# adamchang2000/DenseFusion

Hardware: AMD Instinct MI355X
Metric: poses/sec (node) YCB-Video 1000 pts + 2 refine iters (higher is better)
Workload: dtype f32

## Files before the change

densefusion_amd/csrc/engine.hip:

```cpp
#include <cstdlib>
#include <cstring>
#include <map>
#include <string>
#include <vector>

#include "igemm.h"
#include "layers.h"
#include "wino.h"
#include "pose.h"

namespace df {

struct ParamInfo {
  std::string key;
  int64_t shape[4];
  int ndim;
  int64_t numel() const { int64_t n = 1; for (int i = 0; i < ndim; ++i) n *= shape[i]; return n; }
};

struct Net {
  int kind = 0;
  int num_points = 0, num_obj = 0;
  std::vector<ParamInfo> spec;
  std::map<std::string, int> index;
  std::vector<char> loaded;
  std::map<std::string, float *> buf;
  int device = 0;
  bool profiling = false;
  std::vector<hipEvent_t> ev;
  std::vector<double> ev_flops, ev_bytes, ev_useful;
  std::vector<std::string> ev_desc;
  size_t ev_used = 0;
  bool psp_dirty = false;
  bool upload_pending = false;
  float *stage = nullptr;
  size_t stage_cap = 0;
  bool taps_on = false;
  struct Tap { float *buf = nullptr; size_t cap = 0; int64_t shape[4] = {0, 0, 0, 0}; };
  std::map<std::string, Tap> taps;
};

static void add(Net &n, const std::string &key, std::initializer_list<int64_t> shp) {
  ParamInfo p;
  p.key = key;
  p.ndim = (int)shp.size();
  int i = 0;
  for (auto v : shp) p.shape[i++] = v;
  for (; i < 4; ++i) p.shape[i] = 1;
  n.index[key] = (int)n.spec.size();
  n.spec.push_back(p);
}

static const char *CNN = "cnn.model.module.";

static void build_posenet_spec(Net &n) {
  const std::string c = CNN;
  add(n, c + "feats.conv1.weight", {64, 3, 7, 7});
  int inpl = 64;
  const int planes_of[4] = {64, 128, 256, 512};
  for (int li = 1; li <= 4; ++li) {
    const int planes = planes_of[li - 1];
    for (int blk = 0; blk < 2; ++blk) {
      const int cin = blk == 0 ? inpl : planes;
      const std::string base = c + "feats.layer" + std::to_string(li) + "." + std::to_string(blk) + ".";
      add(n, base + "conv1.weight", {planes, cin, 3, 3});
      add(n, base + "conv2.weight", {planes, planes, 3, 3});
      if (blk == 0 && cin != planes) add(n, base + "downsample.0.weight", {planes, cin, 1, 1});
    }
    inpl = planes;
  }
  for (int s = 0; s < 4; ++s) add(n, c + "psp.stages." + std::to_string(s) + ".1.weight", {512, 512, 1, 1});
  add(n, c + "psp.bottleneck.weight", {1024, 2560, 1, 1});
  add(n, c + "psp.bottleneck.bias", {1024});
  const char *ups[3] = {"up_1", "up_2", "up_3"};
  const int up_in[3] = {1024, 256, 64}, up_out[3] = {256, 64, 64};
  for (int u = 0; u < 3; ++u) {
    add(n, c + ups[u] + ".conv.1.weight", {up_out[u], up_in[u], 3, 3});
    add(n, c + ups[u] + ".conv.1.bias", {up_out[u]});
    add(n, c + ups[u] + ".conv.2.weight", {1});
  }
  add(n, c + "final.0.weight", {32, 64, 1, 1});
  add(n, c + "final.0.bias", {32});
  add(n, c + "classifier.0.weight", {256, 256});
  add(n, c + "classifier.0.bias", {256});
  add(n, c + "classifier.2.weight", {21, 256});
  add(n, c + "classifier.2.bias", {21});
  const char *fn[6] = {"conv1", "conv2", "e_conv1", "e_conv2", "conv5", "conv6"};
  const int fi[6] = {3, 64, 32, 64, 256, 512}, fo[6] = {64, 128, 64, 128, 512, 1024};
  for (int i = 0; i < 6; ++i) {
    add(n, std::string("feat.") + fn[i] + ".weight", {fo[i], fi[i], 1});
    add(n, std::string("feat.") + fn[i] + ".bias", {fo[i]});
  }
  const int hin[3] = {1408, 640, 256}, hout[3] = {640, 256, 128};
  const char *hs[3] = {"r", "t", "c"};
  for (int l = 0; l < 3; ++l)
    for (int h = 0; h < 3; ++h) {
      const std::string nm = "conv" + std::to_string(l + 1) + "_" + hs[h];
      add(n, nm + ".weight", {hout[l], hin[l], 1});
      add(n, nm + ".bias", {hout[l]});
    }
  const int per[3] = {4, 3, 1};
  for (int h = 0; h < 3; ++h) {
    const std::string nm = std::string("conv4_") + hs[h];
    add(n, nm + ".weight", {(int64_t)n.num_obj * per[h], 128, 1});
    add(n, nm + ".bias", {(int64_t)n.num_obj * per[h]});
  }
}

static void build_refiner_spec(Net &n) {
  const char *fn[6] = {"conv1", "conv2", "e_conv1", "e_conv2", "conv5", "conv6"};
  const int fi[6] = {3, 64, 32, 64, 384, 512}, fo[6] = {64, 128, 64, 128, 512, 1024};
  for (int i = 0; i < 6; ++i) {
    add(n, std::string("feat.") + fn[i] + ".weight", {fo[i], fi[i], 1});
    add(n, std::string("feat.") + fn[i] + ".bias", {fo[i]});
  }
  const int li[2] = {1024, 512}, lo[2] = {512, 128};
  const char *hs[2] = {"r", "t"};
  for (int l = 0; l < 2; ++l)
    for (int h = 0; h < 2; ++h) {
      const std::string nm = "conv" + std::to_string(l + 1) + "_" + hs[h];
      add(n, nm + ".weight", {lo[l], li[l]});
      add(n, nm + ".bias", {lo[l]});
    }
  const int per[2] = {4, 3};
  for (int h = 0; h < 2; ++h) {
    const std::string nm = std::string("conv3_") + hs[h];
    add(n, nm + ".weight", {(int64_t)n.num_obj * per[h], 128});
    add(n, nm + ".bias", {(int64_t)n.num_obj * per[h]});
  }
}

static float *dev_alloc(Net &n, const std::string &name, size_t floats) {
  auto it = n.buf.find(name);
  if (it != n.buf.end()) return it->second;
  float *p = nullptr;
  if (hipMalloc(&p, floats * sizeof(float)) != hipSuccess) return nullptr;
  hipMemset(p, 0, floats * sizeof(float));
  n.buf[name] = p;
  return p;
}

__global__ void pack_oihw_kernel(const float *__restrict__ src, float *__restrict__ dst, int O, int I, int HW, int Ipad) {
  const long total = (long)O * HW * Ipad;
  for (long i = blockIdx.x * 256L + threadIdx.x; i < total; i += (long)gridDim.x * 256) {
    const int c = (int)(i % Ipad);
    const long r = i / Ipad;
    const int t = (int)(r % HW);
    const long o = r / HW;
    dst[i] = c < I ? src[(o * I + c) * HW + t] : 0.f;
  }
}

__global__ void psp_fold_kernel(const float *__restrict__ wb, const float *__restrict__ ws, float *__restrict__ wc, int s) {
  const int i = blockIdx.x * 256 + threadIdx.x;
  const int m = blockIdx.y;
  if (i >= 512) return;
  double acc = 0.0;
  for (int o = 0; o < 512; ++o) acc += (double)wb[(size_t)m * 2560 + s * 512 + o] * (double)ws[(size_t)o * 512 + i];
  wc[((size_t)s * 1024 + m) * 512 + i] = (float)acc;
}

static bool ends_with(const std::string &s, const char *suf) {
  const size_t l = strlen(suf);
  return s.size() >= l && s.compare(s.size() - l, l, suf) == 0;
}

static int load_param(Net &n, const std::string &key, const float *src, int64_t numel) {
  auto it = n.index.find(key);
  if (it == n.index.end()) return set_error(DF_ERR_ARG, "load_param: unexpected key '%s'", key.c_str());
  const ParamInfo &pi = n.spec[it->second];
  if (numel != pi.numel())
    return set_error(DF_ERR_ARG, "load_param: size mismatch for %s: got %lld elements, expected %lld", key.c_str(),
                     (long long)numel, (long long)pi.numel());
  if (!src) return set_error(DF_ERR_ARG, "load_param: null pointer for %s", key.c_str());
  hipSetDevice(n.device);
  n.upload_pending = true;
  auto copy = [&](float *dst, const float *s, size_t cnt) { return hipMemcpyAsync(dst, s, cnt * sizeof(float), hipMemcpyDefault, 0); };
  auto copy2d = [&](float *dst, size_t dld, const float *s, size_t sld, size_t width, size_t rows) {
    return hipMemcpy2DAsync(dst, dld * sizeof(float), s, sld * sizeof(float), width * sizeof(float), rows, hipMemcpyDefault, 0);
  };
  hipError_t e = hipSuccess;
  if (pi.ndim == 4 && !ends_with(key, "classifier.0.weight")) {
    const int O = (int)pi.shape[0], I = (int)pi.shape[1], HW = (int)(pi.shape[2] * pi.shape[3]);
    const int Ipad = (I + 3) / 4 * 4;
    float *dst = dev_alloc(n, key, (size_t)O * HW * Ipad);
    if (!dst) return set_error(DF_ERR_LAUNCH, "load_param: hipMalloc failed");
    if (HW == 1 && Ipad == I) e = copy(dst, src, (size_t)numel);
    else {
      if (n.stage_cap < (size_t)numel) {
        if (n.stage) { hipStreamSynchronize(0); hipFree(n.stage); }
        n.stage = nullptr; n.stage_cap = 0;
        if (hipMalloc(&n.stage, (size_t)numel * sizeof(float)) != hipSuccess) return set_error(DF_ERR_LAUNCH, "hipMalloc failed");
        n.stage_cap = (size_t)numel;
      }
      e = copy(n.stage, src, (size_t)numel);
      hipLaunchKernelGGL(pack_oihw_kernel, dim3(256), dim3(256), 0, 0, n.stage, dst, O, I, HW, Ipad);
    }
    if (e == hipSuccess && key.find("feats.layer") != std::string::npos && HW == 9 && I >= 128 && I % 4 == 0 && O % 4 == 0) {
      float *U = dev_alloc(n, key + ".wino", (size_t)16 * O * I), *U4 = dev_alloc(n, key + ".wino4", (size_t)36 * O * I);
      if (!U || !U4) return set_error(DF_ERR_LAUNCH, "load_param: hipMalloc failed");
      launch_wino_weight(dst, U, O, I, 0, 2);
      launch_wino_weight(dst, U4, O, I, 0, 4);
    }
    if (e == hipSuccess && (key.find(".up_1.") != std::string::npos || key.find(".up_2.") != std::string::npos) && HW == 9) {
      float *tm = dev_alloc(n, key + ".tm", (size_t)9 * O * I);
      if (!tm) return set_error(DF_ERR_LAUNCH, "load_param: hipMalloc failed");
      launch_tapmajor(dst, tm, O, I, 0);
    }
  } else if (n.kind == 0 && key.rfind("conv1_", 0) == 0) {
    const int h = key[6] == 'r' ? 0 : key[6] == 't' ? 1 : 2;
    if (ends_with(key, ".weight")) {
      float *wpt = dev_alloc(n, "head1.wpt", (size_t)1920 * 384), *wg = dev_alloc(n, "head1.wg", (size_t)1920 * 1024);
      if (!wpt || !wg) return set_error(DF_ERR_LAUNCH, "hipMalloc failed");
      e = copy2d(wpt + (size_t)h * 640 * 384, 384, src, 1408, 384, 640);
      if (e == hipSuccess) e = copy2d(wg + (size_t)h * 640 * 1024, 1024, src + 384, 1408, 1024, 640);
    } else {
      float *b = dev_alloc(n, "head1.bias", 1920);
      e = copy(b + h * 640, src, 640);
    }
  } else if (n.kind == 0 && (key.rfind("conv2_", 0) == 0 || key.rfind("conv3_", 0) == 0)) {
    const int l = key[4] - '0';
    const int h = key[6] == 'r' ? 0 : key[6] == 't' ? 1 : 2;
    const int co = l == 2 ? 256 : 128, ci = l == 2 ? 640 : 256;
    const std::string nm = std::string("head") + std::to_string(l);
    if (ends_with(key, ".weight")) e = copy(dev_alloc(n, nm + ".w", (size_t)3 * co * ci) + (size_t)h * co * ci, src, (size_t)co * ci);
    else e = copy(dev_alloc(n, nm + ".bias", 3 * co) + h * co, src, co);
  } else if (n.kind == 1 && (key.rfind("conv1_", 0) == 0 || key.rfind("conv2_", 0) == 0)) {
    const int l = key[4] - '0';
    const int h = key[6] == 'r' ? 0 : 1;
    const int co = l == 1 ? 512 : 128, ci = l == 1 ? 1024 : 512;
    const std::string nm = std::string("fc") + std::to_string(l);
    if (ends_with(key, ".weight")) e = copy(dev_alloc(n, nm + ".w", (size_t)2 * co * ci) + (size_t)h * co * ci, src, (size_t)co * ci);
    else e = copy(dev_alloc(n, nm + ".bias", 2 * co) + h * co, src, co);
  } else {
    float *dst = dev_alloc(n, key, (size_t)numel);
    if (!dst) return set_error(DF_ERR_LAUNCH, "load_param: hipMalloc failed");
    e = copy(dst, src, (size_t)numel);
  }
  if (e == hipSuccess && n.kind == 1 && key == "feat.conv5.weight") {
    const float *w5 = n.buf[key];
    float *wx = dev_alloc(n, "feat.conv5.wx", (size_t)512 * 192), *we = dev_alloc(n, "feat.conv5.we", (size_t)512 * 192);
    if (!wx || !we) return set_error(DF_ERR_LAUNCH, "load_param: hipMalloc failed");
    e = copy2d(wx, 192, w5, 384, 64, 512);
    if (e == hipSuccess) e = copy2d(wx + 64, 192, w5 + 128, 384, 128, 512);
    if (e == hipSuccess) e = copy2d(we, 192, w5 + 64, 384, 64, 512);
    if (e == hipSuccess) e = copy2d(we + 64, 192, w5 + 256, 384, 128, 512);
  }
  if (e != hipSuccess) return set_error(DF_ERR_LAUNCH, "load_param(%s): %s", key.c_str(), hipGetErrorString(e));
  n.loaded[it->second] = 1;
  if (n.kind == 0 && key.find(".psp.") != std::string::npos && !ends_with(key, ".bias")) n.psp_dirty = true;
  return DF_OK;
}

static int ensure_derived(Net &n) {
  if (!n.psp_dirty) {
    if (n.upload_pending) {
      if (hipStreamSynchronize(0) != hipSuccess) return set_error(DF_ERR_LAUNCH, "parameter upload failed: %s", hipGetErrorString(hipGetLastError()));
      n.upload_pending = false;
    }
    return DF_OK;
  }
  const std::string P = CNN;
  float *wc = dev_alloc(n, "psp.fold.w", (size_t)4 * 1024 * 512), *wf = dev_alloc(n, "psp.fold.wfeat", (size_t)1024 * 512);
  if (!wc || !wf) return set_error(DF_ERR_LAUNCH, "psp fold: hipMalloc failed");
  const float *wb = n.buf[P + "psp.bottleneck.weight"];
  hipMemcpy2DAsync(wf, 512 * sizeof(float), wb + 2048, 2560 * sizeof(float), 512 * sizeof(float), 1024, hipMemcpyDeviceToDevice, 0);
  for (int st = 0; st < 4; ++st)
    hipLaunchKernelGGL(psp_fold_kernel, dim3(2, 1024, 1), dim3(256), 0, 0, wb, n.buf[P + "psp.stages." + std::to_string(st) + ".1.weight"], wc, st);
  if (hipStreamSynchronize(0) != hipSuccess || check_launch("psp fold") != DF_OK) return DF_ERR_LAUNCH;
  n.psp_dirty = false;
  n.upload_pending = false;
  return DF_OK;
}

static int check_ready(const Net &n0) {
  Net &n = const_cast<Net &>(n0);
  for (size_t i = 0; i < n.spec.size(); ++i)
    if (!n.loaded[i]) return set_error(DF_ERR_STATE, "parameter '%s' was never loaded", n.spec[i].key.c_str());
  return ensure_derived(n);
}

struct Ctx {
  Net *net;
  hipStream_t st;
  bool dry;
  char *base;
  size_t off = 0, cap = 0, peak = 0;
  int err = DF_OK;

  float *f(size_t floats) { return reinterpret_cast<float *>(bytes(floats * sizeof(float))); }
  void *bytes(size_t b) {
    b = (b + 255) & ~size_t(255);
    void *p = dry ? nullptr : base + off;
    off += b;
    if (off > peak) peak = off;
    if (!dry && off > cap && err == DF_OK) err = set_error(DF_ERR_WORKSPACE, "workspace too small: need > %zu bytes, have %zu", off, cap);
    return p;
  }
  bool live() const { return !dry && err == DF_OK; }
  const float *w(const std::string &name) {
    auto it = net->buf.find(name);
    if (it == net->buf.end()) {
      if (err == DF_OK) err = set_error(DF_ERR_STATE, "missing packed parameter '%s'", name.c_str());
      return nullptr;
    }
    return it->second;
  }
  void tap(const char *name, const float *src, int64_t d0, int64_t d1, int64_t d2, int64_t d3) {
    if (!live() || !net->taps_on || !src) return;
    Net::Tap &t = net->taps[name];
    const size_t n = (size_t)d0 * d1 * d2 * d3;
    if (t.cap < n) {
      if (t.buf) hipFree(t.buf);
      t.buf = nullptr; t.cap = 0;
      if (hipMalloc(&t.buf, n * sizeof(float)) != hipSuccess) { (void)hipGetLastError(); return; }
      t.cap = n;
    }
    t.shape[0] = d0; t.shape[1] = d1; t.shape[2] = d2; t.shape[3] = d3;
    hipMemcpyAsync(t.buf, src, n * sizeof(float), hipMemcpyDeviceToDevice, st);
  }
  double pt_useful = 1.0;
  void pconv(const ConvParams &p) { conv(p, pt_useful); }
  void conv(const ConvParams &p, double useful = 1.0) {
    if (!live()) return;
    Net &n = *net;
    if (n.profiling) {
      if (n.ev_used + 2 > n.ev.size()) {
        const size_t old = n.ev.size();
        n.ev.resize(old + 256);
        for (size_t i = old; i < n.ev.size(); ++i) hipEventCreate(&n.ev[i]);
      }
      hipEventRecord(n.ev[n.ev_used], st);
    }
#ifdef DF_DEV
    ConvParams pc = p;
    pc.wgt_const = true;
    const int rc = launch_conv(pc, st);
#else
    const int rc = launch_conv(p, st);
#endif
    if (n.profiling) {
      hipEventRecord(n.ev[n.ev_used + 1], st);
      n.ev_flops.push_back(conv_flops(p));
      n.ev_bytes.push_back(conv_bytes(p));
      n.ev_useful.push_back(conv_flops(p) * useful);
      char d[160];
      snprintf(d, sizeof(d), "M=%ld N=%d K=%d k%dx%d s%d d%d z%d", (long)p.B * p.OH * p.OW, p.Cout, p.KH * p.KW * p.Cin, p.KH,
               p.KW, p.stride, p.dil, p.zcount);
      n.ev_desc.push_back(d);
      n.ev_used += 2;
    }
    if (rc != DF_OK) err = rc;
  }
};

static ConvParams point_gemm(const float *in, int in_ld, int in_coff, int cin, const float *w, const float *bias,
                             float *out, int out_ld, int out_coff, int cout, int rows, int act);

static bool point_fused() {
  static const bool on = df::dev_getenv("DF_POINT_UNFUSED") == nullptr;
  return on;
}

static int wino_route_for(int H, int W, int dil, int ci, int co) {
  static const bool off = df::dev_getenv("DF_NO_WINOGRAD") != nullptr;
  static const int force = df::dev_getenv("DF_WINOGRAD_TILE") ? atoi(df::dev_getenv("DF_WINOGRAD_TILE")) : 0;
  if (off) return 0;
  const int r = wino_route(H, W, dil, ci, co);
  return (r && force == 2) ? 2 : r;
}

static ConvParams point_gemm(const float *in, int in_ld, int in_coff, int cin, const float *w, const float *bias,
                             float *out, int out_ld, int out_coff, int cout, int rows, int act) {
  ConvParams p;
  p.in = in; p.wgt = w; p.bias = bias; p.out = out;
  p.B = rows; p.H = p.W = p.OH = p.OW = 1;
  p.Cin = cin; p.in_ld = in_ld; p.in_coff = in_coff;
  p.Cout = cout; p.out_ld = out_ld; p.out_coff = out_coff;
  p.act = act;
  return p;
}

static ConvParams conv2d(const float *in, int B, int H, int W, int cin, int in_ld, const float *w, const float *bias,
                         float *out, int OH, int OW, int cout, int out_ld, int out_coff, int k, int stride, int pad,
                         int dil, int act) {
  ConvParams p;
  p.in = in; p.wgt = w; p.bias = bias; p.out = out;
  p.B = B; p.H = H; p.W = W; p.OH = OH; p.OW = OW;
  p.Cin = cin; p.in_ld = in_ld; p.Cout = cout; p.out_ld = out_ld; p.out_coff = out_coff;
  p.KH = p.KW = k; p.stride = stride; p.pad = pad; p.dil = dil; p.act = act;
  return p;
}

static inline int conv_out(int in, int k, int stride, int pad, int dil) { return (in + 2 * pad - dil * (k - 1) - 1) / stride + 1; }
static inline int round_up(int v, int m) { return (v + m - 1) / m * m; }

struct PoseNetOut {
  float *out_r, *out_t, *out_c, *emb;
  float *emb_pm = nullptr;
};

struct Grp { int B, H, W; const float *img; };

struct Level {
  std::vector<int> h, w;
  std::vector<long> off;
  long rows = 0;
  void push(int B, int hh, int ww) { h.push_back(hh); w.push_back(ww); off.push_back(rows); rows += (long)B * hh * ww; }
};

static float *cnn_forward(Ctx &c, const std::vector<Grp> &gs, Level &half_lv) {
  const std::string P = CNN;
  const int nb = (int)gs.size();
  Level l0, l1;
  for (const Grp &g : gs) {
    const int H1 = conv_out(g.H, 7, 2, 3, 1), W1 = conv_out(g.W, 7, 2, 3, 1);
    l0.push(g.B, H1, W1);
    l1.push(g.B, conv_out(H1, 3, 2, 1, 1), conv_out(W1, 3, 2, 1, 1));
  }
  float *x = c.f((size_t)l1.rows * 64);
  {
    const size_t mark = c.off;
    for (int i = 0; i < nb; ++i) {
      const Grp &g = gs[i];
      float *img4 = c.f((size_t)g.B * g.H * g.W * 4);
      if (c.live()) launch_nchw3_to_nhwc4(g.img, img4, g.B, g.H, g.W, c.st);
      float *stem = c.f((size_t)g.B * l0.h[i] * l0.w[i] * 64);
      c.conv(conv2d(img4, g.B, g.H, g.W, 4, 4, c.w(P + "feats.conv1.weight"), nullptr, stem, l0.h[i], l0.w[i], 64, 64, 0, 7, 2, 3, 1, ACT_RELU));
      if (c.live()) launch_maxpool3s2(stem, x + l1.off[i] * 64, g.B, l0.h[i], l0.w[i], 64, l1.h[i], l1.w[i], c.st);
      if (nb == 1) c.tap("stem", stem, g.B, l0.h[i], l0.w[i], 64);
    }
    c.off = mark;
    (void)mark;
  }

  auto conv3x3 = [&](const float *in, const Level &li, int ci, const std::string &key, float *out, const Level &lo, int co, int stride, int dil,
                     const float *res) {
    std::vector<int> ws[2];
    for (int i = 0; i < nb; ++i) {
      const int route = stride == 1 ? wino_route_for(li.h[i], li.w[i], dil, ci, co) : 0;
      if (route) { ws[route == 4].push_back(i); continue; }
      ConvParams p = conv2d(in + li.off[i] * ci, gs[i].B, li.h[i], li.w[i], ci, ci, c.w(key), nullptr, out + lo.off[i] * co, lo.h[i], lo.w[i], co,
                            co, 0, 3, stride, dil, dil, ACT_RELU);
      if (res) { p.res = res + lo.off[i] * co; p.res_ld = co; }
      c.conv(p);
    }
    for (int r = 0; r < 2; ++r) {
      if (ws[r].empty()) continue;
      const int m = r ? 4 : 2, nz = (m + 2) * (m + 2);
      std::vector<long> t0;
      long T = 0;
      for (int i : ws[r]) { t0.push_back(T); T += wino_geom(gs[i].B, li.h[i], li.w[i], dil, m).T; }
      const size_t mark = c.off;
      float *V = c.f((size_t)nz * T * ci), *M = c.f((size_t)nz * T * co);
      std::vector<int> tB, tH, tW;
      std::vector<long> trow;
      for (int i : ws[r]) { tB.push_back(gs[i].B); tH.push_back(li.h[i]); tW.push_back(li.w[i]); trow.push_back(li.off[i]); }
      const int nw = (int)ws[r].size();
      static const bool per_bucket = df::dev_getenv("DF_WINO_PER_BUCKET") != nullptr;
      if (m == 4 && !per_bucket) {
        if (c.live()) launch_wino4_input_multi(in, ci, V, nw, tB.data(), tH.data(), tW.data(), trow.data(), t0.data(), ci, dil, T, c.st);
      } else {
        for (size_t j = 0; j < ws[r].size(); ++j) {
          const int i = ws[r][j];
          if (c.live()) launch_wino_input(in + li.off[i] * ci, ci, 0, V, gs[i].B, li.h[i], li.w[i], ci, dil, c.st, T, t0[j], m);
        }
      }
      ConvParams p = point_gemm(V, ci, 0, ci, c.w(key + (r ? ".wino4" : ".wino")), nullptr, M, co, 0, co, (int)T, ACT_NONE);
      p.zcount = nz; p.z_in_coff = T * ci; p.z_wgt = (long)co * ci; p.z_out_coff = T * co;
      double px = 0;
      for (int i : ws[r]) px += (double)gs[i].B * li.h[i] * li.w[i];
      c.conv(p, px / ((double)(m * m) * (double)T));
      if (m == 4 && !per_bucket) {
        if (c.live()) launch_wino4_output_multi(M, out, co, res, co, ACT_RELU, nw, tB.data(), tH.data(), tW.data(), trow.data(), t0.data(), co, dil, T, c.st);
      } else {
        for (size_t j = 0; j < ws[r].size(); ++j) {
          const int i = ws[r][j];
          if (c.live())
            launch_wino_output(M, out + lo.off[i] * co, co, 0, nullptr, res ? res + lo.off[i] * co : nullptr, co, 0, ACT_RELU, gs[i].B, li.h[i], li.w[i],
                               co, dil, c.st, T, t0[j], m);
        }
      }
      c.off = mark;
    }
  };

  Level lx = l1;
  int cin = 64;
  const int planes_of[4] = {64, 128, 256, 512}, stride_of[4] = {1, 2, 1, 1}, dil_of[4] = {1, 1, 2, 4};
  for (int li = 1; li <= 4; ++li) {
    const int planes = planes_of[li - 1], s = stride_of[li - 1], d = dil_of[li - 1];
    const std::string base = P + "feats.layer" + std::to_string(li) + ".";
    Level lo;
    for (int i = 0; i < nb; ++i) lo.push(gs[i].B, conv_out(lx.h[i], 3, s, 1, 1), conv_out(lx.w[i], 3, s, 1, 1));
    float *t = c.f((size_t)lo.rows * planes);
    conv3x3(x, lx, cin, base + "0.conv1.weight", t, lo, planes, s, 1, nullptr);
    const float *res = x;
    if (cin != planes || s != 1) {
      float *ds = c.f((size_t)lo.rows * planes);
      if (s == 1) {
        c.conv(point_gemm(x, cin, 0, cin, c.w(base + "0.downsample.0.weight"), nullptr, ds, planes, 0, planes, (int)lo.rows, ACT_NONE));
      } else {
        for (int i = 0; i < nb; ++i)
          c.conv(conv2d(x + lx.off[i] * cin, gs[i].B, lx.h[i], lx.w[i], cin, cin, c.w(base + "0.downsample.0.weight"), nullptr, ds + lo.off[i] * planes,
                        lo.h[i], lo.w[i], planes, planes, 0, 1, s, 0, 1, ACT_NONE));
      }
      res = ds;
    }
    float *o0 = c.f((size_t)lo.rows * planes);
    conv3x3(t, lo, planes, base + "0.conv2.weight", o0, lo, planes, 1, 1, res);
    float *t1 = c.f((size_t)lo.rows * planes);
    conv3x3(o0, lo, planes, base + "1.conv1.weight", t1, lo, planes, 1, d, nullptr);
    float *o1 = c.f((size_t)lo.rows * planes);
    conv3x3(t1, lo, planes, base + "1.conv2.weight", o1, lo, planes, 1, d, o0);
    x = o1; lx = lo; cin = planes;
    if (nb == 1) c.tap(("layer" + std::to_string(li)).c_str(), x, gs[0].B, lx.h[0], lx.w[0], planes);
  }
  float *prior = c.f((size_t)lx.rows * 1024);
  for (int i = 0; i < nb; ++i) {
    const int B = gs[i].B;
    float *pooled = c.f((size_t)4 * B * 36 * 512), *zst = c.f((size_t)4 * B * 36 * 1024);
    if (c.live()) launch_psp_pool(x + lx.off[i] * 512, 512, 0, pooled, B, lx.h[i], lx.w[i], 512, c.st);
    ConvParams p = point_gemm(pooled, 512, 0, 512, c.w("psp.fold.w"), nullptr, zst, 1024, 0, 1024, B * 36, ACT_NONE);
    p.zcount = 4; p.z_in_coff = (long)B * 36 * 512; p.z_wgt = 1024 * 512; p.z_out_coff = (long)B * 36 * 1024;
    c.conv(p);
    if (c.live()) launch_psp_prior_sum(zst, prior + lx.off[i] * 1024, B, lx.h[i], lx.w[i], 1024, c.st);
  }
  float *psp = c.f((size_t)lx.rows * 1024);
  {
    ConvParams p = point_gemm(x, 512, 0, 512, c.w("psp.fold.wfeat"), c.w(P + "psp.bottleneck.bias"), psp, 1024, 0, 1024, (int)lx.rows, ACT_RELU);
    p.res = prior; p.res_ld = 1024;
    c.conv(p);
  }
  if (nb == 1) c.tap("psp", psp, gs[0].B, lx.h[0], lx.w[0], 1024);
  float *cur = psp;
  const char *ups[2] = {"up_1", "up_2"};
  const int up_in[2] = {1024, 256}, up_out[2] = {256, 64};
  for (int u = 0; u < 2; ++u) {
    const size_t mark = c.off;
    float *o = c.f((size_t)4 * lx.rows * up_out[u]);
    const size_t keep = c.off;
    float *y = c.f((size_t)lx.rows * 9 * up_out[u]);
    c.conv(point_gemm(cur, up_in[u], 0, up_in[u], c.w(P + ups[u] + ".conv.1.weight.tm"), nullptr, y, 9 * up_out[u], 0, 9 * up_out[u], (int)lx.rows,
                      ACT_NONE));
    Level lo;
    for (int i = 0; i < nb; ++i) lo.push(gs[i].B, 2 * lx.h[i], 2 * lx.w[i]);
    for (int i = 0; i < nb; ++i)
      if (c.live()) {
        const int rc = launch_upconv_gather(y + lx.off[i] * 9 * up_out[u], c.w(P + ups[u] + ".conv.1.bias"), c.w(P + ups[u] + ".conv.2.weight"),
                                            o + lo.off[i] * up_out[u], gs[i].B, lx.h[i], lx.w[i], up_out[u], c.st);
        if (rc != DF_OK) c.err = rc;
      }
    c.off = keep;
    (void)mark;
    lx = lo;
    cur = o;
    if (nb == 1) c.tap(ups[u], cur, gs[0].B, lx.h[0], lx.w[0], up_out[u]);
  }
  half_lv = lx;
  return cur;
}

struct SelectOut { double *pose_wo, *state; float *rt; };

static void posenet_points(Ctx &c, int B, int N, int Npad, const float *cloud, const float *emb_pm, const int64_t *obj,
                           float *out_r, float *out_t, float *out_c, const SelectOut *sel = nullptr) {
  Net &n = *c.net;
  const int rows = B * Npad;
  float *pf = c.f((size_t)rows * 384);
  if (point_fused()) {
    PointFeatParams q;
    q.cloud = cloud; q.emb = emb_pm; q.pf = pf; q.ld = 384; q.cx1 = 0; q.ce1 = 64; q.cx2 = 128; q.ce2 = 256;
    q.w1 = c.w("feat.conv1.weight"); q.b1 = c.w("feat.conv1.bias"); q.w2 = c.w("feat.conv2.weight"); q.b2 = c.w("feat.conv2.bias");
    q.we1 = c.w("feat.e_conv1.weight"); q.be1 = c.w("feat.e_conv1.bias"); q.we2 = c.w("feat.e_conv2.weight"); q.be2 = c.w("feat.e_conv2.bias");
    q.B = B; q.N = N; q.Npad = Npad;
    if (c.live()) { const int rc = launch_pointfeat(q, c.st); if (rc != DF_OK) c.err = rc; }
  } else {
    if (c.live()) launch_cloud_conv1(cloud, nullptr, c.w("feat.conv1.weight"), c.w("feat.conv1.bias"), pf, 384, B, N, Npad, c.st);
    c.pconv(point_gemm(emb_pm, 32, 0, 32, c.w("feat.e_conv1.weight"), c.w("feat.e_conv1.bias"), pf, 384, 64, 64, rows, ACT_RELU));
    c.pconv(point_gemm(pf, 384, 0, 64, c.w("feat.conv2.weight"), c.w("feat.conv2.bias"), pf, 384, 128, 128, rows, ACT_RELU));
    c.pconv(point_gemm(pf, 384, 64, 64, c.w("feat.e_conv2.weight"), c.w("feat.e_conv2.bias"), pf, 384, 256, 128, rows, ACT_RELU));
  }
  float *x5 = c.f((size_t)rows * 512);
  c.pconv(point_gemm(pf, 384, 128, 256, c.w("feat.conv5.weight"), c.w("feat.conv5.bias"), x5, 512, 0, 512, rows, ACT_RELU));
  ConvParams p6 = point_gemm(x5, 512, 0, 512, c.w("feat.conv6.weight"), c.w("feat.conv6.bias"), nullptr, 1024, 0, 1024, rows, ACT_RELU);
  p6.rows_per_group = Npad; p6.rows_valid = N;
  const int prow = conv_colsum_rows(p6);
  float *partial = c.f((size_t)prow * 1024);
  p6.colsum = partial;
  c.pconv(p6);
  float *apx = c.f((size_t)B * 1024);
  if (c.live()) launch_colsum_finish(partial, prow / B, apx, B, 1024, N, c.st);
  c.tap("ap_x", apx, B, 1024, 1, 1);
  float *gbias = c.f((size_t)B * 1920);
  if (c.live()) launch_fc_rows(apx, 1024, 0, c.w("head1.wg"), c.w("head1.bias"), gbias, 1920, B, 1024, 1920, 1, 0, c.st);
  if (sel) {
    float *h1c = c.f((size_t)rows * 640), *h2c = c.f((size_t)rows * 256), *h3c = c.f((size_t)rows * 128), *conf = c.f((size_t)B * N);
    const float *w1 = c.w("head1.wpt"), *w2 = c.w("head2.w"), *b2 = c.w("head2.bias"), *w3 = c.w("head3.w"), *b3 = c.w("head3.bias");
    if (c.err != DF_OK) return;
    {
      ConvParams p = point_gemm(pf, 384, 0, 384, c.dry ? nullptr : w1 + (size_t)2 * 640 * 384, c.dry ? nullptr : gbias + 1280, h1c, 640, 0, 640, rows, ACT_RELU);
      p.rows_per_group = Npad; p.rows_valid = N; p.bias_group_ld = 1920;
      c.pconv(p);
    }
    c.pconv(point_gemm(h1c, 640, 0, 640, c.dry ? nullptr : w2 + (size_t)2 * 256 * 640, c.dry ? nullptr : b2 + 512, h2c, 256, 0, 256, rows, ACT_RELU));
    c.pconv(point_gemm(h2c, 256, 0, 256, c.dry ? nullptr : w3 + (size_t)2 * 128 * 256, c.dry ? nullptr : b3 + 256, h3c, 128, 0, 128, rows, ACT_RELU));
    if (c.live())
      launch_head_select(h3c, c.w("conv4_c.weight"), c.w("conv4_c.bias"), pf, gbias, w1, w2, b2, w3, b3, c.w("conv4_r.weight"),
                         c.w("conv4_r.bias"), c.w("conv4_t.weight"), c.w("conv4_t.bias"), obj, n.num_obj, cloud, B, N, Npad, conf, sel->pose_wo,
                         sel->state, sel->rt, nullptr, c.st);
    return;
  }
  float *h1 = c.f((size_t)rows * 1920);
  {
    ConvParams p = point_gemm(pf, 384, 0, 384, c.w("head1.wpt"), gbias, h1, 1920, 0, 1920, rows, ACT_RELU);
    p.rows_per_group = Npad; p.rows_valid = N; p.bias_group_ld = 1920;
    c.pconv(p);
  }
  float *h2 = c.f((size_t)rows * 768), *h3 = c.f((size_t)rows * 384);
  {
    ConvParams p = point_gemm(h1, 1920, 0, 640, c.w("head2.w"), c.w("head2.bias"), h2, 768, 0, 256, rows, ACT_RELU);
    p.zcount = 3; p.z_in_coff = 640; p.z_wgt = 256 * 640; p.z_bias = 256; p.z_out_coff = 256;
    c.pconv(p);
  }
  {
    ConvParams p = point_gemm(h2, 768, 0, 256, c.w("head3.w"), c.w("head3.bias"), h3, 384, 0, 128, rows, ACT_RELU);
    p.zcount = 3; p.z_in_coff = 256; p.z_wgt = 128 * 256; p.z_bias = 128; p.z_out_coff = 128;
    c.pconv(p);
  }
  if (c.live())
    launch_head_final(h3, c.w("conv4_r.weight"), c.w("conv4_r.bias"), c.w("conv4_t.weight"), c.w("conv4_t.bias"),
                      c.w("conv4_c.weight"), c.w("conv4_c.bias"), obj, n.num_obj, out_r, out_t, out_c, B, N, Npad, c.st);
}

static void posenet_forward(Ctx &c, const std::vector<Grp> &gs, const float *cloud, const int64_t *choose, const int64_t *obj, PoseNetOut &o,
                            const SelectOut *sel = nullptr) {
  const int N = c.net->num_points, Npad = round_up(N, 128);
  c.pt_useful = (double)N / Npad;
  int B = 0;
  for (const Grp &g : gs) B += g.B;
  Level hl;
  float *half = cnn_forward(c, gs, hl);
  const std::string P = CNN;
  float *patch = c.f((size_t)B * Npad * 576), *z3 = c.f((size_t)B * Npad * 64);
  {
    long b0 = 0;
    for (size_t i = 0; i < gs.size(); ++i) {
      if (c.live())
        launch_up3_patches(half + hl.off[i] * 64, choose + b0 * N, patch + (size_t)b0 * Npad * 576, gs[i].B, hl.h[i], hl.w[i], N, Npad, c.st);
      b0 += gs[i].B;
    }
  }
  {
    ConvParams p = point_gemm(patch, 576, 0, 576, c.w(P + "up_3.conv.1.weight"), c.w(P + "up_3.conv.1.bias"), z3, 64, 0, 64, B * Npad, ACT_PRELU);
    p.prelu = c.w(P + "up_3.conv.2.weight");
    c.pconv(p);
  }
  if (gs.size() == 1) c.tap("up_3", z3, B, Npad, 64, 1);
  o.emb_pm = c.f((size_t)B * Npad * 32);
  if (c.live()) launch_final_logsoftmax(z3, c.w(P + "final.0.weight"), c.w(P + "final.0.bias"), o.emb, o.emb_pm, B, N, Npad, c.st);
  posenet_points(c, B, N, Npad, cloud, o.emb_pm, obj, o.out_r, o.out_t, o.out_c, sel);
}

struct RefinerBufs { float *pf, *e5, *x5, *partial, *apx, *f1, *f2; int prow; };

static RefinerBufs refiner_alloc(Ctx &c, int B, int N, int Npad) {
  RefinerBufs r;
  c.pt_useful = (double)N / Npad;
  const int rows = B * Npad;
  r.pf = c.f((size_t)rows * 384);
  r.e5 = c.f((size_t)rows * 512);
  r.x5 = c.f((size_t)rows * 512);
  ConvParams p6 = point_gemm(r.x5, 512, 0, 512, nullptr, nullptr, nullptr, 1024, 0, 1024, rows, ACT_RELU);
  p6.rows_per_group = Npad; p6.rows_valid = N;
  r.prow = conv_colsum_rows(p6);
  r.partial = c.f((size_t)r.prow * 1024);
  r.apx = c.f((size_t)B * 1024);
  r.f1 = c.f((size_t)B * 1024);
  r.f2 = c.f((size_t)B * 256);
  return r;
}

static void refiner_prepare(Ctx &c, const RefinerBufs &r, int B, int Npad, const float *emb_pm) {
  const int rows = B * Npad;
  if (point_fused()) {
    PointFeatParams q;
    q.emb = emb_pm; q.pf = r.pf; q.ld = 384; q.ce1 = 192; q.ce2 = 256;
    q.we1 = c.w("feat.e_conv1.weight"); q.be1 = c.w("feat.e_conv1.bias"); q.we2 = c.w("feat.e_conv2.weight"); q.be2 = c.w("feat.e_conv2.bias");
    q.B = B; q.N = c.net->num_points; q.Npad = Npad;
    if (c.live()) { const int rc = launch_pointfeat(q, c.st); if (rc != DF_OK) c.err = rc; }
  } else {
    c.pconv(point_gemm(emb_pm, 32, 0, 32, c.w("feat.e_conv1.weight"), c.w("feat.e_conv1.bias"), r.pf, 384, 192, 64, rows, ACT_RELU));
    c.pconv(point_gemm(r.pf, 384, 192, 64, c.w("feat.e_conv2.weight"), c.w("feat.e_conv2.bias"), r.pf, 384, 256, 128, rows, ACT_RELU));
  }
  c.pconv(point_gemm(r.pf, 384, 192, 192, c.w("feat.conv5.we"), c.w("feat.conv5.bias"), r.e5, 512, 0, 512, rows, ACT_NONE));
}

static void refiner_iterate(Ctx &c, const RefinerBufs &r, int B, int N, int Npad, const float *cloud, const float *rt,
                            const int64_t *obj, float *out_r, float *out_t, double *state, float *rt_next, double *pose_out) {
  const int rows = B * Npad;
  if (point_fused()) {
    PointFeatParams q;
    q.cloud = cloud; q.rt = rt; q.pf = r.pf; q.ld = 384; q.cx1 = 0; q.cx2 = 64;
    q.w1 = c.w("feat.conv1.weight"); q.b1 = c.w("feat.conv1.bias"); q.w2 = c.w("feat.conv2.weight"); q.b2 = c.w("feat.conv2.bias");
    q.B = B; q.N = N; q.Npad = Npad;
    if (c.live()) { const int rc = launch_pointfeat(q, c.st); if (rc != DF_OK) c.err = rc; }
  } else {
    if (c.live()) launch_cloud_conv1(cloud, rt, c.w("feat.conv1.weight"), c.w("feat.conv1.bias"), r.pf, 384, B, N, Npad, c.st);
    c.pconv(point_gemm(r.pf, 384, 0, 64, c.w("feat.conv2.weight"), c.w("feat.conv2.bias"), r.pf, 384, 64, 128, rows, ACT_RELU));
  }
  {
    ConvParams p = point_gemm(r.pf, 384, 0, 192, c.w("feat.conv5.wx"), nullptr, r.x5, 512, 0, 512, rows, ACT_RELU);
    p.res = r.e5; p.res_ld = 512;
    c.pconv(p);
  }
  ConvParams p6 = point_gemm(r.x5, 512, 0, 512, c.w("feat.conv6.weight"), c.w("feat.conv6.bias"), nullptr, 1024, 0, 1024, rows, ACT_RELU);
  p6.rows_per_group = Npad; p6.rows_valid = N; p6.colsum = r.partial;
  c.pconv(p6);
  if (c.live()) launch_colsum_finish(r.partial, r.prow / B, r.apx, B, 1024, N, c.st);
  if (c.live()) {
    launch_fc_rows(r.apx, 1024, 0, c.w("fc1.w"), c.w("fc1.bias"), r.f1, 1024, B, 1024, 1024, 1, 1, c.st);
    launch_fc_rows(r.f1, 1024, 512, c.w("fc2.w"), c.w("fc2.bias"), r.f2, 256, B, 512, 128, 2, 1, c.st);
  }
  if (c.live()) {
    launch_refiner_tail(r.f2, c.w("conv3_r.weight"), c.w("conv3_r.bias"), c.w("conv3_t.weight"), c.w("conv3_t.bias"), obj,
                        c.net->num_obj, out_r, out_t, state, rt_next, pose_out, B, c.st);
  }
}

static Net *as_net(df_net *h) { return reinterpret_cast<Net *>(h); }
static const Net *as_net(const df_net *h) { return reinterpret_cast<const Net *>(h); }

static int finish(Ctx &c, const char *what) {
  if (c.err != DF_OK) return c.err;
  return c.dry ? DF_OK : check_launch(what);
}

}

using namespace df;

extern "C" df_net *df_posenet_create(int num_points, int num_obj) {
  if (num_points <= 0 || num_obj <= 0) { set_error(DF_ERR_ARG, "posenet_create: bad sizes"); return nullptr; }
  Net *n = new Net();
  n->kind = 0; n->num_points = num_points; n->num_obj = num_obj;
  hipGetDevice(&n->device);
  build_posenet_spec(*n);
  n->loaded.assign(n->spec.size(), 0);
  return reinterpret_cast<df_net *>(n);
}

extern "C" df_net *df_refiner_create(int num_points, int num_obj) {
  if (num_points <= 0 || num_obj <= 0) { set_error(DF_ERR_ARG, "refiner_create: bad sizes"); return nullptr; }
  Net *n = new Net();
  n->kind = 1; n->num_points = num_points; n->num_obj = num_obj;
  hipGetDevice(&n->device);
  build_refiner_spec(*n);
  n->loaded.assign(n->spec.size(), 0);
  return reinterpret_cast<df_net *>(n);
}

extern "C" void df_net_destroy(df_net *h) {
  if (!h) return;
  Net *n = as_net(h);
#ifdef DF_DEV
  split_gemm_invalidate();
#endif
  for (auto &kv : n->buf) hipFree(kv.second);
  if (n->stage) hipFree(n->stage);
  for (auto &kv : n->taps) if (kv.second.buf) hipFree(kv.second.buf);
  for (auto e : n->ev) hipEventDestroy(e);
  delete n;
}

extern "C" int df_net_num_params(const df_net *h) { return h ? (int)as_net(h)->spec.size() : 0; }

extern "C" int df_net_param_info(const df_net *h, int i, char *key_out, int key_cap, int64_t *shape4, int *ndim) {
// ... 32 lines not shown
  if (!h) return set_error(DF_ERR_ARG, "profile_read: null handle");
  Net *n = as_net(h);
  double ms = 0, fl = 0, by = 0, us = 0;
  static const bool verbose = df::dev_getenv("DF_PROFILE_VERBOSE") != nullptr;
  for (size_t i = 0; i + 1 < n->ev_used; i += 2) {
    float t = 0;
    if (hipEventElapsedTime(&t, n->ev[i], n->ev[i + 1]) != hipSuccess) return set_error(DF_ERR_LAUNCH, "profile_read: events not complete");
    ms += t;
    fl += n->ev_flops[i / 2];
    by += n->ev_bytes[i / 2];
    us += n->ev_useful[i / 2];
    if (verbose)
      fprintf(stderr, "[df-gemm] %s  %.1f us  %.1f TFLOP/s\n", n->ev_desc[i / 2].c_str(), t * 1e3, n->ev_flops[i / 2] / t / 1e9);
  }
  if (gemm_ms) *gemm_ms = ms;
  if (gemm_flops) *gemm_flops = fl;
  if (gemm_useful_flops) *gemm_useful_flops = us;
  if (gemm_bytes) *gemm_bytes = by;
  if (launches) *launches = (int)(n->ev_used / 2);
  n->ev_used = 0;
  n->ev_flops.clear();
  n->ev_bytes.clear();
  n->ev_useful.clear();
  n->ev_desc.clear();
  return DF_OK;
}

extern "C" int df_net_debug_taps(df_net *h, int enable) {
  if (!h) return set_error(DF_ERR_ARG, "debug_taps: null handle");
  Net *n = as_net(h);
  n->taps_on = enable != 0;
  if (!enable) {
    for (auto &kv : n->taps) if (kv.second.buf) hipFree(kv.second.buf);
    n->taps.clear();
  }
  return DF_OK;
}

extern "C" int df_net_debug_tap_read(df_net *h, const char *name, float *dst, int64_t cap, int64_t *shape4) {
  if (!h || !name) return set_error(DF_ERR_ARG, "debug_tap_read: null handle / name");
  Net *n = as_net(h);
  auto it = n->taps.find(name);
  if (it == n->taps.end() || !it->second.buf) return set_error(DF_ERR_STATE, "debug_tap_read: no tap named '%s' (arm df_net_debug_taps and run a single-bucket forward)", name);
  const Net::Tap &t = it->second;
  const int64_t numel = t.shape[0] * t.shape[1] * t.shape[2] * t.shape[3];
  if (shape4) for (int i = 0; i < 4; ++i) shape4[i] = t.shape[i];
  if (!dst) return DF_OK;
  if (cap < numel) return set_error(DF_ERR_ARG, "debug_tap_read: destination holds %lld floats, tap '%s' has %lld", (long long)cap, name, (long long)numel);
  if (hipMemcpy(dst, t.buf, (size_t)numel * sizeof(float), hipMemcpyDefault) != hipSuccess) return set_error(DF_ERR_LAUNCH, "debug_tap_read: copy failed");
  return DF_OK;
}

static int posenet_args_ok(const Net *n, int B, int H, int W) {
  if (!n || n->kind != 0) return set_error(DF_ERR_ARG, "not a PoseNet handle");
  if (B <= 0 || H < 8 || W < 8) return set_error(DF_ERR_ARG, "posenet: need B >= 1 and H, W >= 8 (got %d, %d, %d)", B, H, W);
  if (H > DF_MAX_CROP || W > DF_MAX_CROP) return set_error(DF_ERR_ARG, "posenet: crops beyond %d pixels per side are not supported (got %d x %d)", DF_MAX_CROP, H, W);
  return DF_OK;
}

static int make_groups(const Net *n, int nb, const int *B, const int *H, const int *W, const float *const *img, std::vector<Grp> &gs) {
  if (nb <= 0 || nb > 4096 || !B || !H || !W) return set_error(DF_ERR_ARG, "need 1..4096 buckets with B / H / W arrays (got nb = %d)", nb);
  long tot = 0;
  gs.clear();
  for (int i = 0; i < nb; ++i) {
    const int rc = posenet_args_ok(n, B[i], H[i], W[i]);
    if (rc != DF_OK) return rc;
    if (img && !img[i]) return set_error(DF_ERR_ARG, "bucket %d: null image pointer", i);
    gs.push_back(Grp{B[i], H[i], W[i], img ? img[i] : nullptr});
    tot += B[i];
  }
  if (tot > (1 << 20)) return set_error(DF_ERR_ARG, "too many objects in one call (%ld)", tot);
  return DF_OK;
}

extern "C" size_t df_posenet_workspace_bytes(const df_net *h, int B, int H, int W) {
  if (posenet_args_ok(as_net(h), B, H, W) != DF_OK) return 0;
  Ctx c{const_cast<Net *>(as_net(h)), nullptr, true, nullptr};
  PoseNetOut o{};
  posenet_forward(c, {Grp{B, H, W, nullptr}}, nullptr, nullptr, nullptr, o);
  return c.peak;
}

extern "C" int df_posenet_forward(df_net *h, int B, int H, int W, const float *img, const float *cloud,
                                  const int64_t *choose, const int64_t *obj, float *out_r, float *out_t, float *out_c,
                                  float *emb, void *ws, size_t ws_bytes, df_stream_t stream) {
  int rc = posenet_args_ok(as_net(h), B, H, W);
  if (rc != DF_OK) return rc;
  if ((rc = check_ready(*as_net(h))) != DF_OK) return rc;
  if (!img || !cloud || !choose || !obj || !out_r || !out_t || !out_c || !emb || !ws) return set_error(DF_ERR_ARG, "posenet_forward: null pointer");
  Ctx c{as_net(h), to_stream(stream), false, static_cast<char *>(ws)};
  c.cap = ws_bytes;
  if (df_posenet_workspace_bytes(h, B, H, W) > ws_bytes) return set_error(DF_ERR_WORKSPACE, "posenet_forward: workspace too small");
  PoseNetOut o{out_r, out_t, out_c, emb};
  posenet_forward(c, {Grp{B, H, W, img}}, cloud, choose, obj, o);
  return finish(c, "posenet_forward");
}

extern "C" size_t df_posenet_multi_workspace_bytes(const df_net *h, int nb, const int *B, const int *H, const int *W) {
  std::vector<Grp> gs;
  if (!h || as_net(h)->kind != 0 || make_groups(as_net(h), nb, B, H, W, nullptr, gs) != DF_OK) return 0;
  Ctx c{const_cast<Net *>(as_net(h)), nullptr, true, nullptr};
  PoseNetOut o{};
  posenet_forward(c, gs, nullptr, nullptr, nullptr, o);
  return c.peak;
}

extern "C" int df_posenet_forward_multi(df_net *h, int nb, const int *B, const int *H, const int *W, const float *const *img, const float *cloud,
                                        const int64_t *choose, const int64_t *obj, float *out_r, float *out_t, float *out_c, float *emb, void *ws,
                                        size_t ws_bytes, df_stream_t stream) {
  if (!h || as_net(h)->kind != 0) return set_error(DF_ERR_ARG, "not a PoseNet handle");
  if (!img) return set_error(DF_ERR_ARG, "posenet_forward_multi: null pointer");
  std::vector<Grp> gs;
  int rc = make_groups(as_net(h), nb, B, H, W, img, gs);
  if (rc != DF_OK) return rc;
  if ((rc = check_ready(*as_net(h))) != DF_OK) return rc;
  if (!cloud || !choose || !obj || !out_r || !out_t || !out_c || !emb || !ws) return set_error(DF_ERR_ARG, "posenet_forward_multi: null pointer");
  if (df_posenet_multi_workspace_bytes(h, nb, B, H, W) > ws_bytes) return set_error(DF_ERR_WORKSPACE, "posenet_forward_multi: workspace too small");
  Ctx c{as_net(h), to_stream(stream), false, static_cast<char *>(ws)};
  c.cap = ws_bytes;
  PoseNetOut o{out_r, out_t, out_c, emb};
  posenet_forward(c, gs, cloud, choose, obj, o);
  return finish(c, "posenet_forward_multi");
}

static void refiner_standalone(Ctx &c, int B, const float *x, const float *emb, const int64_t *obj, float *out_r, float *out_t) {
  const int N = c.net->num_points, Npad = round_up(N, 128);
  float *emb_pm = c.f((size_t)B * Npad * 32);
  RefinerBufs r = refiner_alloc(c, B, N, Npad);
  if (c.live()) launch_emb_to_pm(emb, emb_pm, B, N, Npad, c.st);
  refiner_prepare(c, r, B, Npad, emb_pm);
  refiner_iterate(c, r, B, N, Npad, x, nullptr, obj, out_r, out_t, nullptr, nullptr, nullptr);
}

extern "C" size_t df_refiner_workspace_bytes(const df_net *h, int B) {
  if (!h || as_net(h)->kind != 1 || B <= 0) return 0;
  Ctx c{const_cast<Net *>(as_net(h)), nullptr, true, nullptr};
  refiner_standalone(c, B, nullptr, nullptr, nullptr, nullptr, nullptr);
  return c.peak;
}

extern "C" int df_refiner_forward(df_net *h, int B, const float *x, const float *emb, const int64_t *obj, float *out_r,
                                  float *out_t, void *ws, size_t ws_bytes, df_stream_t stream) {
  if (!h || as_net(h)->kind != 1) return set_error(DF_ERR_ARG, "not a PoseRefineNet handle");
  if (B <= 0) return set_error(DF_ERR_ARG, "refiner_forward: B must be >= 1");
  int rc = check_ready(*as_net(h));
  if (rc != DF_OK) return rc;
  if (!x || !emb || !obj || !out_r || !out_t || !ws) return set_error(DF_ERR_ARG, "refiner_forward: null pointer");
  if (df_refiner_workspace_bytes(h, B) > ws_bytes) return set_error(DF_ERR_WORKSPACE, "refiner_forward: workspace too small");
  Ctx c{as_net(h), to_stream(stream), false, static_cast<char *>(ws)};
  c.cap = ws_bytes;
  refiner_standalone(c, B, x, emb, obj, out_r, out_t);
  return finish(c, "refiner_forward");
}

static void estimate(Ctx &cp, Ctx &cr, const std::vector<Grp> &gs, const float *cloud, const int64_t *choose, const int64_t *obj, int iters,
                     double *pose_wo, double *pose) {
  const int N = cp.net->num_points, Npad = round_up(N, 128);
  int B = 0;
  for (const Grp &g : gs) B += g.B;
  PoseNetOut o{};
  o.emb = cp.f((size_t)B * 32 * N);
  double *state = reinterpret_cast<double *>(cp.bytes((size_t)B * 7 * sizeof(double)));
  float *rt = cp.f((size_t)B * 12);
  const SelectOut sel{pose_wo, state, rt};
  posenet_forward(cp, gs, cloud, choose, obj, o, &sel);
  cr.off = cp.off;
  cr.peak = cp.peak;
  RefinerBufs r = refiner_alloc(cr, B, N, Npad);
  if (iters > 0) refiner_prepare(cr, r, B, Npad, o.emb_pm);
  for (int it = 0; it < iters; ++it)
    refiner_iterate(cr, r, B, N, Npad, cloud, rt, obj, nullptr, nullptr, state, rt, it == iters - 1 ? pose : nullptr);
  if (iters == 0 && cp.live() && pose) hipMemcpyAsync(pose, state, (size_t)B * 7 * sizeof(double), hipMemcpyDeviceToDevice, cp.st);
}

static int estimate_handles_ok(const df_net *pn, const df_net *rf) {
  if (!pn || as_net(pn)->kind != 0) return set_error(DF_ERR_ARG, "estimate_poses: not a PoseNet handle");
  if (!rf || as_net(rf)->kind != 1) return set_error(DF_ERR_ARG, "estimate_poses: not a PoseRefineNet handle");
  if (as_net(rf)->num_points != as_net(pn)->num_points || as_net(rf)->num_obj != as_net(pn)->num_obj)
    return set_error(DF_ERR_ARG, "estimate_poses: estimator / refiner disagree on num_points or num_obj");
  return DF_OK;
}

extern "C" size_t df_estimate_multi_workspace_bytes(const df_net *pn, const df_net *rf, int nb, const int *B, const int *H, const int *W) {
  std::vector<Grp> gs;
  if (estimate_handles_ok(pn, rf) != DF_OK || make_groups(as_net(pn), nb, B, H, W, nullptr, gs) != DF_OK) return 0;
  Ctx cp{const_cast<Net *>(as_net(pn)), nullptr, true, nullptr}, cr{const_cast<Net *>(as_net(rf)), nullptr, true, nullptr};
  estimate(cp, cr, gs, nullptr, nullptr, nullptr, 1, nullptr, nullptr);
  return cr.peak;
}

extern "C" int df_estimate_poses_multi(df_net *pn, df_net *rf, int nb, const int *B, const int *H, const int *W, const float *const *img,
                                       const float *cloud, const int64_t *choose, const int64_t *obj, int iters, double *pose_wo,
                                       double *pose, void *ws, size_t ws_bytes, df_stream_t stream) {
  int rc = estimate_handles_ok(pn, rf);
  if (rc != DF_OK) return rc;
  std::vector<Grp> gs;
  if (!img) return set_error(DF_ERR_ARG, "estimate_poses: null pointer");
  if ((rc = make_groups(as_net(pn), nb, B, H, W, img, gs)) != DF_OK) return rc;
  if (iters < 0) return set_error(DF_ERR_ARG, "estimate_poses: iters < 0");
  if ((rc = check_ready(*as_net(pn))) != DF_OK || (rc = check_ready(*as_net(rf))) != DF_OK) return rc;
  if (!cloud || !choose || !obj || !pose || !ws) return set_error(DF_ERR_ARG, "estimate_poses: null pointer");
  if (df_estimate_multi_workspace_bytes(pn, rf, nb, B, H, W) > ws_bytes) return set_error(DF_ERR_WORKSPACE, "estimate_poses: workspace too small");
  Ctx cp{as_net(pn), to_stream(stream), false, static_cast<char *>(ws)}, cr{as_net(rf), to_stream(stream), false, static_cast<char *>(ws)};
  cp.cap = cr.cap = ws_bytes;
  estimate(cp, cr, gs, cloud, choose, obj, iters, pose_wo, pose);
  if (cp.err != DF_OK) return cp.err;
  return finish(cr, "estimate_poses");
}

extern "C" size_t df_estimate_workspace_bytes(const df_net *pn, const df_net *rf, int B, int H, int W) {
  return df_estimate_multi_workspace_bytes(pn, rf, 1, &B, &H, &W);
}

extern "C" int df_estimate_poses(df_net *pn, df_net *rf, int B, int H, int W, const float *img, const float *cloud,
                                 const int64_t *choose, const int64_t *obj, int iters, double *pose_wo, double *pose,
                                 void *ws, size_t ws_bytes, df_stream_t stream) {
  return df_estimate_poses_multi(pn, rf, 1, &B, &H, &W, &img, cloud, choose, obj, iters, pose_wo, pose, ws, ws_bytes, stream);
}

static int conv_desc_to_params(const df_conv_desc *d, ConvParams &p, const char *what);

static thread_local int t_last_splitk = 1;
extern "C" int df_conv_last_splitk(void) { return t_last_splitk; }

extern "C" int df_conv2d_nhwc(const df_conv_desc *d, df_stream_t stream) {
  if (!d) return set_error(DF_ERR_ARG, "conv2d_nhwc: null descriptor");
  if (d->KH != d->KW) return set_error(DF_ERR_ARG, "conv2d_nhwc: square kernels only");
  if (d->act == ACT_PRELU && !d->prelu) return set_error(DF_ERR_ARG, "conv2d_nhwc: PReLU needs a slope");
  ConvParams p;
  p.in = d->in; p.wgt = d->wgt; p.bias = d->bias; p.res = d->res; p.prelu = d->prelu; p.out = d->out;
  p.B = d->B; p.H = d->H; p.W = d->W; p.Cin = d->Cin; p.in_ld = d->in_ld; p.in_coff = d->in_coff;
  p.OH = d->OH; p.OW = d->OW; p.Cout = d->Cout; p.out_ld = d->out_ld; p.out_coff = d->out_coff;
  p.res_ld = d->res_ld; p.res_coff = d->res_coff;
  p.KH = d->KH; p.KW = d->KW; p.stride = d->stride; p.pad = d->pad; p.dil = d->dil; p.act = d->act;
  if (p.OH != conv_out(p.H, p.KH, p.stride, p.pad, p.dil) || p.OW != conv_out(p.W, p.KW, p.stride, p.pad, p.dil))
    return set_error(DF_ERR_ARG, "conv2d_nhwc: OH/OW do not match the convolution geometry");
  p.splitk_ws = static_cast<float *>(d->splitk_ws); p.splitk_ws_bytes = d->splitk_ws ? d->splitk_ws_bytes : 0;
  return launch_conv(p, to_stream(stream), &t_last_splitk);
}

static int make_segs(const df_conv_desc *d, int nb, const int *B, const int *H, const int *W, std::vector<WgradSeg> &segs, const char *what) {
  if (!d) return set_error(DF_ERR_ARG, "%s: null descriptor", what);
  if (nb <= 0 || nb > 4096 || !B || !H || !W) return set_error(DF_ERR_ARG, "%s: need 1..4096 buckets with B / H / W arrays", what);
  if (d->KH != d->KW) return set_error(DF_ERR_ARG, "%s: square kernels only", what);
  long in_row = 0, out_row = 0;
  for (int i = 0; i < nb; ++i) {
    if (B[i] <= 0 || H[i] <= 0 || W[i] <= 0) return set_error(DF_ERR_ARG, "%s: bucket %d is empty", what, i);
    const int OH = conv_out(H[i], d->KH, d->stride, d->pad, d->dil), OW = conv_out(W[i], d->KW, d->stride, d->pad, d->dil);
    if (OH <= 0 || OW <= 0) return set_error(DF_ERR_ARG, "%s: bucket %d: the kernel does not fit the map", what, i);
    segs.push_back(WgradSeg{B[i], H[i], W[i], OH, OW, in_row, out_row});
    in_row += (long)B[i] * H[i] * W[i];
    out_row += (long)B[i] * OH * OW;
  }
  return DF_OK;
}

extern "C" int df_conv2d_nhwc_multi(const df_conv_desc *d, int nb, const int *B, const int *H, const int *W, df_stream_t stream) {
  std::vector<WgradSeg> segs;
  int rc = make_segs(d, nb, B, H, W, segs, "conv2d_nhwc_multi");
  if (rc != DF_OK) return rc;
  if (d->act == ACT_PRELU && !d->prelu) return set_error(DF_ERR_ARG, "conv2d_nhwc_multi: PReLU needs a slope");
  ConvParams p;
  p.in = d->in; p.wgt = d->wgt; p.bias = d->bias; p.res = d->res; p.prelu = d->prelu; p.out = d->out;
  p.Cin = d->Cin; p.in_ld = d->in_ld; p.in_coff = d->in_coff; p.Cout = d->Cout; p.out_ld = d->out_ld; p.out_coff = d->out_coff;
  p.res_ld = d->res_ld; p.res_coff = d->res_coff;
  p.KH = d->KH; p.KW = d->KW; p.stride = d->stride; p.pad = d->pad; p.dil = d->dil; p.act = d->act;
  return launch_conv_multi(p, nb, segs.data(), to_stream(stream));
}

extern "C" size_t df_conv2d_wgrad_multi_workspace_bytes(const df_conv_desc *d, int nb, const int *B, const int *H, const int *W) {
  std::vector<WgradSeg> segs;
  if (make_segs(d, nb, B, H, W, segs, "conv2d_wgrad_multi_workspace_bytes") != DF_OK) return 0;
  ConvParams p;
  p.Cin = d->Cin; p.Cout = d->Cout; p.KH = d->KH; p.KW = d->KW;
  return wgrad_multi_workspace_bytes(p, nb, segs.data());
}

extern "C" int df_conv2d_wgrad_nhwc_multi(const df_conv_desc *d, int nb, const int *B, const int *H, const int *W, const float *dy, float *dw, float *db,
                                          void *ws, size_t ws_bytes, df_stream_t stream) {
  std::vector<WgradSeg> segs;
  int rc = make_segs(d, nb, B, H, W, segs, "conv2d_wgrad_multi");
  if (rc != DF_OK) return rc;
  if (!dy || !dw || !d->in) return set_error(DF_ERR_ARG, "conv2d_wgrad_multi: null pointer");
  ConvParams p;
  p.in = d->in; p.out = const_cast<float *>(dy);
  p.Cin = d->Cin; p.in_ld = d->in_ld; p.in_coff = d->in_coff; p.Cout = d->Cout; p.out_ld = d->out_ld; p.out_coff = d->out_coff;
  p.KH = d->KH; p.KW = d->KW; p.stride = d->stride; p.pad = d->pad; p.dil = d->dil;
  return launch_wgrad_multi(p, nb, segs.data(), dw, db, ws, ws_bytes, to_stream(stream));
}

static int wino_desc_ok(const df_conv_desc *d, const char *what) {
  if (!d) return set_error(DF_ERR_ARG, "%s: null descriptor", what);
  if (d->KH != 3 || d->KW != 3 || d->stride != 1 || d->pad != d->dil || d->dil < 1)
    return set_error(DF_ERR_ARG, "%s: needs a 3x3 kernel, stride 1, pad == dil", what);
  if (d->Cin % 4 || d->Cout % 4 || d->in_ld % 4 || d->in_coff % 4 || d->out_ld % 4 || d->out_coff % 4 || d->B <= 0 || d->H <= 0 || d->W <= 0)
    return set_error(DF_ERR_ARG, "%s: channel counts / strides must be multiples of 4", what);
  if (d->OH != d->H || d->OW != d->W) return set_error(DF_ERR_ARG, "%s: OH/OW must equal H/W", what);
  if (d->act != ACT_NONE && d->act != ACT_RELU) return set_error(DF_ERR_ARG, "%s: activation must be none or ReLU", what);
  return DF_OK;
}

extern "C" size_t df_conv3x3_winograd_tile_scratch_bytes(const df_conv_desc *d, int tile) {
  if (wino_desc_ok(d, "conv3x3_winograd_scratch_bytes") != DF_OK) return 0;
  if (tile != 2 && tile != 4) { set_error(DF_ERR_ARG, "conv3x3_winograd: tile must be 2 or 4"); return 0; }
  const WinoGeom g = wino_geom(d->B, d->H, d->W, d->dil, tile);
  const size_t nz = (size_t)(tile + 2) * (tile + 2);
  return (nz * d->Cout * d->Cin + nz * g.T * d->Cin + nz * g.T * d->Cout) * sizeof(float);
}

extern "C" int df_conv3x3_winograd_tile_nhwc(const df_conv_desc *d, int tile, void *scratch, size_t scratch_bytes, df_stream_t stream) {
  int rc = wino_desc_ok(d, "conv3x3_winograd_nhwc");
  if (rc != DF_OK) return rc;
  if (tile != 2 && tile != 4) return set_error(DF_ERR_ARG, "conv3x3_winograd: tile must be 2 or 4");
  if (!d->in || !d->wgt || !d->out || !scratch) return set_error(DF_ERR_ARG, "conv3x3_winograd_nhwc: null pointer");
  if (scratch_bytes < df_conv3x3_winograd_tile_scratch_bytes(d, tile)) return set_error(DF_ERR_WORKSPACE, "conv3x3_winograd_nhwc: scratch too small");
  const WinoGeom g = wino_geom(d->B, d->H, d->W, d->dil, tile);
  const int nz = (tile + 2) * (tile + 2);
  hipStream_t st = to_stream(stream);
  float *U = static_cast<float *>(scratch), *V = U + (size_t)nz * d->Cout * d->Cin, *M = V + (size_t)nz * g.T * d->Cin;
  launch_wino_weight(d->wgt, U, d->Cout, d->Cin, st, tile);
  launch_wino_input(d->in, d->in_ld, d->in_coff, V, d->B, d->H, d->W, d->Cin, d->dil, st, 0, 0, tile);
  ConvParams p;
  p.in = V; p.wgt = U; p.out = M;
  p.B = (int)g.T; p.Cin = d->Cin; p.in_ld = d->Cin; p.Cout = d->Cout; p.out_ld = d->Cout;
  p.zcount = nz; p.z_in_coff = g.T * d->Cin; p.z_wgt = (long)d->Cout * d->Cin; p.z_out_coff = g.T * d->Cout;
  rc = launch_conv(p, st);
  if (rc != DF_OK) return rc;
  launch_wino_output(M, d->out, d->out_ld, d->out_coff, d->bias, d->res, d->res_ld, d->res_coff, d->act, d->B, d->H, d->W, d->Cout, d->dil, st, 0, 0,
                     tile);
  return check_launch("conv3x3_winograd_nhwc");
}

extern "C" int df_wino_route(int H, int W, int dil, int Cin, int Cout) { return wino_route(H, W, dil, Cin, Cout); }

extern "C" size_t df_conv3x3_winograd_scratch_bytes(const df_conv_desc *d) { return df_conv3x3_winograd_tile_scratch_bytes(d, 2); }

extern "C" int df_conv3x3_winograd_nhwc(const df_conv_desc *d, void *scratch, size_t scratch_bytes, df_stream_t stream) {
  return df_conv3x3_winograd_tile_nhwc(d, 2, scratch, scratch_bytes, stream);
}

namespace df {
__global__ void flip_transpose_kernel(const float *__restrict__ w, float *__restrict__ wt, int O, int T, int I, int KH, int KW) {
  const long total = (long)O * T * I;
  for (long i = blockIdx.x * 256L + threadIdx.x; i < total; i += (long)gridDim.x * 256) {
    const int n = (int)(i % O);
    const long r = i / O;
    const int t = (int)(r % T);
    const long c = r / T;
    const int ky = t / KW, kx = t - ky * KW;
    const int tf = (KH - 1 - ky) * KW + (KW - 1 - kx);
    wt[i] = w[((size_t)n * T + tf) * I + c];
  }
}
}

static int conv_desc_to_params(const df_conv_desc *d, ConvParams &p, const char *what) {
  if (!d) return set_error(DF_ERR_ARG, "%s: null descriptor", what);
  if (d->KH != d->KW) return set_error(DF_ERR_ARG, "%s: square kernels only", what);
  p.in = d->in; p.wgt = d->wgt; p.bias = d->bias; p.res = d->res; p.prelu = d->prelu; p.out = d->out;
  p.B = d->B; p.H = d->H; p.W = d->W; p.Cin = d->Cin; p.in_ld = d->in_ld; p.in_coff = d->in_coff;
  p.OH = d->OH; p.OW = d->OW; p.Cout = d->Cout; p.out_ld = d->out_ld; p.out_coff = d->out_coff;
  p.res_ld = d->res_ld; p.res_coff = d->res_coff;
  p.KH = d->KH; p.KW = d->KW; p.stride = d->stride; p.pad = d->pad; p.dil = d->dil; p.act = d->act;
  if (p.OH != conv_out(p.H, p.KH, p.stride, p.pad, p.dil) || p.OW != conv_out(p.W, p.KW, p.stride, p.pad, p.dil))
    return set_error(DF_ERR_ARG, "%s: OH/OW do not match the convolution geometry", what);
  return DF_OK;
}

extern "C" int df_conv2d_dgrad_nhwc(const df_conv_desc *d, const float *dy, float *dx, float *w_scratch, int accumulate,
                                    df_stream_t stream) {
  ConvParams f;
  int rc = conv_desc_to_params(d, f, "conv2d_dgrad");
  if (rc != DF_OK) return rc;
  if (!dy || !dx || !w_scratch || !f.wgt) return set_error(DF_ERR_ARG, "conv2d_dgrad: null pointer");
  if (f.Cout % 4) return set_error(DF_ERR_ARG, "conv2d_dgrad: Cout must be a multiple of 4");
  hipStream_t st = to_stream(stream);
  const int T = f.KH * f.KW;
  hipLaunchKernelGGL(flip_transpose_kernel, dim3(256), dim3(256), 0, st, f.wgt, w_scratch, f.Cout, T, f.Cin, f.KH, f.KW);
  ConvParams q;
  q.in = dy; q.B = f.B; q.H = f.OH; q.W = f.OW; q.Cin = f.Cout; q.in_ld = f.out_ld; q.in_coff = f.out_coff;
  q.wgt = w_scratch;
  q.out = dx; q.OH = f.H; q.OW = f.W; q.Cout = f.Cin; q.out_ld = f.in_ld; q.out_coff = f.in_coff;
  q.KH = f.KH; q.KW = f.KW; q.stride = 1; q.up = f.stride; q.dil = f.dil; q.pad = f.dil * (f.KH - 1) - f.pad;
  if (q.pad < 0) return set_error(DF_ERR_ARG, "conv2d_dgrad: padding larger than the kernel reach is not supported");
  if (accumulate) { q.res = dx; q.res_ld = f.in_ld; q.res_coff = f.in_coff; }
  q.splitk_ws = static_cast<float *>(d->splitk_ws); q.splitk_ws_bytes = d->splitk_ws ? d->splitk_ws_bytes : 0;
  return launch_conv(q, st, &t_last_splitk);
}

extern "C" size_t df_conv2d_wgrad_workspace_bytes(const df_conv_desc *d) {
  ConvParams f;
  if (conv_desc_to_params(d, f, "conv2d_wgrad_workspace_bytes") != DF_OK) return 0;
  return wgrad_workspace_bytes(f);
}

extern "C" int df_conv2d_wgrad_nhwc(const df_conv_desc *d, const float *dy, float *dw, float *db, void *ws, size_t ws_bytes, df_stream_t stream) {
  ConvParams f;
  int rc = conv_desc_to_params(d, f, "conv2d_wgrad");
  if (rc != DF_OK) return rc;
  if (!dy || !dw || !f.in) return set_error(DF_ERR_ARG, "conv2d_wgrad: null pointer");
  f.out = const_cast<float *>(dy);
  return launch_wgrad(f, dw, db, ws, ws_bytes, to_stream(stream));
}
```

densefusion_amd/csrc/train.hip:

```cpp
#include <algorithm>
#include <cstdlib>
#include <cstring>
#include <deque>
#include <functional>
#include <map>
#include <memory>
#include <string>
#include <vector>

#include "igemm.h"
#include "loss.h"
#include "layers.h"
#include "wino.h"

namespace df {
namespace {

typedef float f32x4 __attribute__((ext_vector_type(4)));
constexpr int TB = 256;
inline unsigned nblk(long n, long cap = 16384) { long b = (n + TB - 1) / TB; return (unsigned)(b < 1 ? 1 : (b > cap ? cap : b)); }
#define GRID_STRIDE(i, n) for (long i = blockIdx.x * (long)TB + threadIdx.x; i < (n); i += (long)gridDim.x * TB)
inline int round_up(int v, int m) { return (v + m - 1) / m * m; }
inline int conv_out(int in, int k, int stride, int pad, int dil) { return (in + 2 * pad - dil * (k - 1) - 1) / stride + 1; }

// ... 1151 lines not shown
void build_refiner(Trainer &t) {
  add_plain(t, "feat.conv1.weight", {64, 3, 1});
  add_plain(t, "feat.conv1.bias", {64});
  const char *fn[5] = {"conv2", "e_conv1", "e_conv2", "conv5", "conv6"};
  const int fi[5] = {64, 32, 64, 384, 512}, fo[5] = {128, 64, 128, 512, 1024};
  for (int i = 0; i < 5; ++i) {
    add_gemm(t, std::string("feat.") + fn[i] + ".weight", fo[i], fi[i], true);
    add_plain(t, std::string("feat.") + fn[i] + ".bias", {fo[i]});
  }
  const int li[2] = {1024, 512}, lo[2] = {512, 128};
  const char *hs[2] = {"r", "t"};
  for (int l = 0; l < 2; ++l)
    for (int h = 0; h < 2; ++h) {
      const std::string nm = "conv" + std::to_string(l + 1) + "_" + hs[h];
      add_gemm(t, nm + ".weight", lo[l], li[l], false);
      add_plain(t, nm + ".bias", {lo[l]});
    }
  const int per[2] = {4, 3};
  for (int h = 0; h < 2; ++h) {
    const std::string nm = std::string("conv3_") + hs[h];
    add_plain(t, nm + ".weight", {(int64_t)t.K * per[h], 128});
    add_plain(t, nm + ".bias", {(int64_t)t.K * per[h]});
  }
}

struct View { float *d = nullptr; int ld = 0; };

struct Lv {
  std::vector<int> B, H, W;
  std::vector<long> off;
  std::vector<int> b0;
  long rows = 0;
  int frames = 0;
  int nb() const { return (int)B.size(); }
  void push(int b, int h, int w) {
    B.push_back(b); H.push_back(h); W.push_back(w); off.push_back(rows); b0.push_back(frames);
    rows += (long)b * h * w; frames += b;
  }
};

struct Act {
  View v, g;
  const Lv *lv = nullptr;
  int C = 0;
  bool gset = false;
  long rows() const { return lv->rows; }
};

enum GemmKind { GK_FWD = 0, GK_DGRAD = 1, GK_WGRAD = 2 };

struct Step {
  Trainer *t;
  hipStream_t st;
  bool dry;
  char *base;
  size_t off = 0, cap = 0, peak = 0;
  int err = DF_OK;
  const float *P = nullptr;
  float *G = nullptr;
  float *splitk = nullptr;
  size_t splitk_bytes = 0;
  std::deque<Act> acts;
  std::deque<Lv> lvs;
  std::vector<std::function<void()>> tape;
#ifdef DF_DEV
  hipStream_t side = nullptr;
  hipEvent_t ev_fork = nullptr, ev_join = nullptr;
  bool keep_wgrad_ws = false;
#endif

  void *bytes(size_t b) {
    b = (b + 255) & ~size_t(255);
    void *p = (dry ? reinterpret_cast<char *>(4096) : base) + off;
    off += b;
    if (off > peak) peak = off;
    if (!dry && off > cap && err == DF_OK) err = set_error(DF_ERR_WORKSPACE, "train step: workspace too small (need > %zu bytes, have %zu)", off, cap);
    return p;
  }
  float *f(size_t n) { return static_cast<float *>(bytes(n * sizeof(float))); }
  bool live() const { return !dry && err == DF_OK; }
#ifdef DF_DEV
  void dbg(const char *what, const std::string &extra = std::string()) {
    static const bool on = df::dev_getenv("DF_TRAIN_DEBUG") != nullptr;
    if (!on || dry) return;
    const hipError_t e = hipStreamSynchronize(st);
    fprintf(stderr, "[df-train] %s %s: %s\n", what, extra.c_str(), e == hipSuccess ? "ok" : hipGetErrorString(e));
    fflush(stderr);
  }
#else
  void dbg(const char *, const std::string & = std::string()) {}
#endif
  void fail(int rc) { if (rc != DF_OK && err == DF_OK) err = rc; }
  void prof_begin() {
    if (!t->profiling || !live()) return;
    if (t->ev_used + 2 > t->ev.size()) {
      const size_t old = t->ev.size();
      t->ev.resize(old + 512);
      for (size_t i = old; i < t->ev.size(); ++i) hipEventCreate(&t->ev[i]);
    }
    hipEventRecord(t->ev[t->ev_used], st);
  }
  void prof_end(int kind, double flops, const ConvParams *p = nullptr, long M = 0) {
    if (!t->profiling || !live()) return;
    hipEventRecord(t->ev[t->ev_used + 1], st);
    t->ev_kind.push_back(kind);
    t->ev_flops.push_back(flops);
#ifdef DF_DEV
    char d[160] = "";
    if (p) snprintf(d, sizeof(d), "M=%ld N=%d K=%d k%dx%d s%d d%d z%d", M > 0 ? M : (long)p->B * p->OH * p->OW, p->Cout, p->KH * p->KW * p->Cin, p->KH, p->KW, p->stride, p->dil, p->zcount);
    t->ev_desc.push_back(d);
#endif
    t->ev_used += 2;
  }
  void gemm(int kind, const ConvParams &p) {
    if (!live()) return;
    prof_begin();
    fail(launch_conv(p, st));
    prof_end(kind, conv_flops(p), &p);
  }
  void gemm_multi(int kind, const ConvParams &p, const std::vector<WgradSeg> &segs) {
    if (!live() || segs.empty()) return;
    double fl = 0;
    for (const WgradSeg &g : segs) fl += 2.0 * g.B * g.OH * g.OW * (double)p.Cout * p.KH * p.KW * p.Cin;
    prof_begin();
    fail(launch_conv_multi(p, (int)segs.size(), segs.data(), st));
    long M = 0;
    for (const WgradSeg &g : segs) M += (long)g.B * g.OH * g.OW;
    prof_end(kind, fl, &p, M);
  }
  size_t slot(const std::string &name) {
    auto it = t->slot.find(name);
    if (it == t->slot.end()) {
      if (err == DF_OK) err = set_error(DF_ERR_STATE, "trainer: no parameter slot named '%s'", name.c_str());
      return 0;
    }
    return it->second;
  }
  const float *p(const std::string &name, size_t extra = 0) { const size_t o = slot(name); return dry ? nullptr : P + o + extra; }
  float *gr(const std::string &name, size_t extra = 0) { const size_t o = slot(name); return dry ? nullptr : G + o + extra; }
  const float *pf(const std::string &name, size_t extra = 0) { const size_t o = slot(name); return dry ? nullptr : t->wflip + o + extra; }
  const Lv *level(const Lv &l) { lvs.push_back(l); return &lvs.back(); }
  const Lv *flat_level(long rows) { Lv l; l.push((int)rows, 1, 1); return level(l); }
  Act *act(const Lv *lv, int C, float *d = nullptr, int ld = 0) {
    acts.emplace_back();
    Act *a = &acts.back();
    a->lv = lv; a->C = C;
    a->v.d = d ? d : f((size_t)lv->rows * C);
    a->v.ld = d ? ld : C;
    return a;
  }
  Act *act(long rows, int C, float *d = nullptr, int ld = 0) { return act(flat_level(rows), C, d, ld); }
  bool grad_of(Act *a) {
    if (!a->g.d) { a->g.d = f((size_t)a->rows() * a->C); a->g.ld = a->C; }
    const bool acc = a->gset;
    a->gset = true;
    return acc;
  }
};

ConvParams flat_params(const Act *x, int cin, const float *w, const float *bias, Act *y, int act) {
  ConvParams p;
  p.in = x->v.d; p.wgt = w; p.bias = bias; p.out = y->v.d;
  p.B = (int)x->rows(); p.H = p.W = p.OH = p.OW = 1; p.Cin = cin; p.in_ld = x->v.ld;
  p.Cout = y->C; p.out_ld = y->v.ld;
  p.act = act;
  return p;
}
std::vector<BTab> make_tabs(const Lv *lv, const Lv *aux = nullptr) {
  std::vector<BTab> out;
  for (int g0 = 0; g0 < lv->nb(); g0 += TAB_MAX) {
    BTab t{};
    t.n = std::min(TAB_MAX, lv->nb() - g0);
    for (int i = 0; i < TAB_MAX; ++i) {
      const int g = g0 + std::min(i, t.n - 1);
      t.B[i] = lv->B[g]; t.H[i] = lv->H[g]; t.W[i] = lv->W[g]; t.b0[i] = lv->b0[g];
      t.row0[i] = lv->off[g]; t.row1[i] = lv->off[g] + (long)lv->B[g] * lv->H[g] * lv->W[g];
      t.aux0[i] = aux ? aux->off[g] : 0;
    }
    out.push_back(t);
  }
  return out;
}
inline long tab_rows(const BTab &t) { return t.row1[t.n - 1] - t.row0[0]; }
inline int tab_frames(const BTab &t) { return t.b0[t.n - 1] + t.B[t.n - 1] - t.b0[0]; }

ConvParams bucket_params(const Act *x, int i, int cin, const float *w, const float *bias, Act *y, int k, int stride, int pad, int dil, int act) {
  ConvParams p;
  const Lv *li = x->lv, *lo = y->lv;
  p.in = x->v.d + li->off[i] * x->v.ld; p.wgt = w; p.bias = bias; p.out = y->v.d + lo->off[i] * y->v.ld;
  p.B = li->B[i]; p.H = li->H[i]; p.W = li->W[i]; p.Cin = cin; p.in_ld = x->v.ld;
  p.OH = lo->H[i]; p.OW = lo->W[i]; p.Cout = y->C; p.out_ld = y->v.ld;
  p.KH = p.KW = k; p.stride = stride; p.pad = pad; p.dil = dil; p.act = act;
  return p;
}

void launch_act_bwd(Step &s, Act *y, int act, const float *slope, float *dslope) {
  const long rows = y->rows();
  const int C4 = y->C / 4;
  const unsigned blocks = act == 2 ? nblk(rows * C4, 512) : nblk(rows * C4);
  float *part = act == 2 ? s.f(blocks) : nullptr;
  if (!s.live()) return;
  hipLaunchKernelGGL(act_bwd2d_kernel, dim3(blocks), dim3(TB), 0, s.st, y->g.d, y->g.ld, y->v.d, y->v.ld, rows, C4, act, slope, part);
  if (act == 2) hipLaunchKernelGGL(sum_partials_kernel, dim3(1), dim3(TB), 0, s.st, part, (int)blocks, 1L, dslope, 1);
}

void wgrad(Step &s, ConvParams f, const std::vector<WgradSeg> &segs, View gy, float *dw, float *db) {
  f.out = gy.d; f.out_ld = gy.ld; f.out_coff = 0;
  f.bias = nullptr; f.res = nullptr; f.act = ACT_NONE; f.zcount = 1;
  f.rows_per_group = f.rows_valid = f.bias_group_ld = 0;
  const size_t mark = s.off;
  const size_t need = wgrad_multi_workspace_bytes(f, (int)segs.size(), segs.data());
  void *ws = s.bytes(need);
  hipStream_t st = s.st;
  bool keep = false;
#ifdef DF_DEV
  keep = s.keep_wgrad_ws;
  if (keep && s.live() && s.side) {
    hipEventRecord(s.ev_fork, s.st);
    hipStreamWaitEvent(s.side, s.ev_fork, 0);
    st = s.side;
  }
#endif
  if (s.live()) {
    double M = 0;
    for (const WgradSeg &g : segs) M += (double)g.B * g.OH * g.OW;
    s.prof_begin();
    s.fail(launch_wgrad_multi(f, (int)segs.size(), segs.data(), dw, db, ws, need, st, 1));
    s.prof_end(GK_WGRAD, 2.0 * M * f.Cout * f.KH * f.KW * f.Cin, &f, (long)M);
  }
#ifdef DF_DEV
  if (keep && s.live() && s.side) {
    hipEventRecord(s.ev_join, s.side);
    static const bool sync_dbg = df::dev_getenv("DF_TRAIN_OVERLAP_SYNC") != nullptr;
    if (sync_dbg) hipStreamSynchronize(s.side);
  }
#endif
  s.dbg("wgrad");
  if (!keep) s.off = mark;
}
void wgrad(Step &s, const ConvParams &f, View gy, float *dw, float *db) {
  wgrad(s, f, std::vector<WgradSeg>{WgradSeg{f.B, f.H, f.W, f.OH, f.OW, 0, 0}}, gy, dw, db);
}

void dgrad(Step &s, const ConvParams &f, View gy, View dx, const float *wflip, bool accumulate) {
  ConvParams q;
  q.in = gy.d; q.B = f.B; q.H = f.OH; q.W = f.OW; q.Cin = f.Cout; q.in_ld = gy.ld;
  q.wgt = wflip;
  q.out = dx.d; q.OH = f.H; q.OW = f.W; q.Cout = f.Cin; q.out_ld = dx.ld;
  q.KH = f.KH; q.KW = f.KW; q.stride = 1; q.up = f.stride; q.dil = f.dil; q.pad = f.dil * (f.KH - 1) - f.pad;
  if (accumulate) { q.res = dx.d; q.res_ld = dx.ld; }
  if (f.zcount > 1) {
    q.zcount = f.zcount; q.z_in_coff = f.z_out_coff; q.z_out_coff = f.z_in_coff; q.z_wgt = (long)f.Cin * f.Cout * f.KH * f.KW;
  }
  q.splitk_ws = s.splitk; q.splitk_ws_bytes = s.splitk_bytes;
  s.gemm(GK_DGRAD, q);
  s.dbg("dgrad");
}

struct ConvW {
  std::string name;
  size_t woff = 0;
  std::string bias;
  size_t boff = 0;
  std::string slope;
};

View rows_view(View v, long row0) { return View{v.d + row0 * v.ld, v.ld}; }

Act *conv(Step &s, Act *x, int cin, const ConvW &cw, int cout, int k, int stride, int pad, int dil, int act, Act *res = nullptr, Act *into = nullptr,
          bool need_dx = true) {
  const Lv *li = x->lv;
  const int nb = li->nb();
  const bool flat = k == 1 && stride == 1 && pad == 0;
  const Lv *lo = li;
  if (!flat) {
    Lv o;
    for (int i = 0; i < nb; ++i) o.push(li->B[i], conv_out(li->H[i], k, stride, pad, dil), conv_out(li->W[i], k, stride, pad, dil));
    lo = s.level(o);
  }
  Act *y = into ? into : s.act(lo, cout);
  if (!flat && into) y->lv = lo;
  const float *wp = s.p(cw.name, cw.woff), *bp = cw.bias.empty() ? nullptr : s.p(cw.bias, cw.boff);
  const float *slope = act == ACT_PRELU ? s.p(cw.slope) : nullptr;
  auto plan = std::make_shared<std::vector<ConvParams>>();
  auto f4 = std::make_shared<std::vector<int>>();
  const auto wit = s.t->wino.find(cw.name);
  const bool wino_ok = !flat && wit != s.t->wino.end() && k == 3 && stride == 1 && pad == dil && cw.bias.empty() && act != ACT_PRELU;
  if (flat) {
    ConvParams p = flat_params(x, cin, wp, bp, y, act);
    if (res) { p.res = res->v.d; p.res_ld = res->v.ld; }
    p.prelu = slope;
    p.splitk_ws = s.splitk; p.splitk_ws_bytes = s.splitk_bytes;
    plan->push_back(p);
    s.gemm(GK_FWD, p);
  } else {
    std::vector<WgradSeg> direct;
    int first_direct = -1;
    for (int i = 0; i < nb; ++i) {
      ConvParams p = bucket_params(x, i, cin, wp, bp, y, k, stride, pad, dil, act);
      if (res) { p.res = res->v.d + lo->off[i] * res->v.ld; p.res_ld = res->v.ld; }
      p.prelu = slope;
      p.splitk_ws = s.splitk; p.splitk_ws_bytes = s.splitk_bytes;
      plan->push_back(p);
      if (wino_ok && wino_route(li->H[i], li->W[i], dil, cin, cout) == 4) { f4->push_back(i); continue; }
      if (first_direct < 0) first_direct = i;
      direct.push_back(WgradSeg{li->B[i], li->H[i], li->W[i], lo->H[i], lo->W[i], li->off[i], lo->off[i]});
    }
    if (direct.size() == 1) s.gemm(GK_FWD, (*plan)[first_direct]);
    else if (!direct.empty()) {
      ConvParams p = (*plan)[0];
      p.in = x->v.d; p.out = y->v.d;
      if (res) p.res = res->v.d;
      s.gemm_multi(GK_FWD, p, direct);
    }
  }
  auto wino_pass = [=](Step &s, View in, int ci, const float *U, View out, int co, const float *rs, int rs_ld, int a, int kind) {
    if (f4->empty()) return;
    std::vector<int> tB, tH, tW;
    std::vector<long> trow, t0;
    long T = 0;
    for (int i : *f4) {
      tB.push_back(li->B[i]); tH.push_back(li->H[i]); tW.push_back(li->W[i]); trow.push_back(li->off[i]);
      t0.push_back(T);
      T += wino_geom(li->B[i], li->H[i], li->W[i], dil, 4).T;
    }
    const size_t mark = s.off;
    float *V = s.f((size_t)36 * T * ci), *M = s.f((size_t)36 * T * co);
    if (s.live()) {
      const int nw = (int)f4->size();
      launch_wino4_input_multi(in.d, in.ld, V, nw, tB.data(), tH.data(), tW.data(), trow.data(), t0.data(), ci, dil, T, s.st);
      ConvParams q;
      q.in = V; q.wgt = U; q.out = M;
      q.B = (int)T; q.Cin = ci; q.in_ld = ci; q.Cout = co; q.out_ld = co;
      q.zcount = 36; q.z_in_coff = T * ci; q.z_wgt = (long)co * ci; q.z_out_coff = T * co;
      s.gemm(kind, q);
      launch_wino4_output_multi(M, out.d, out.ld, rs, rs_ld, a, nw, tB.data(), tH.data(), tW.data(), trow.data(), t0.data(), co, dil, T, s.st);
    }
    s.off = mark;
  };
  wino_pass(s, x->v, cin, s.dry || !wino_ok ? nullptr : s.t->wino_buf + wit->second.fwd, y->v, cout, res ? res->v.d : nullptr, res ? res->v.ld : 0, act, GK_FWD);
  s.dbg("conv fwd", cw.name);
  Step *sp = &s;
  s.tape.push_back([=]() {
    Step &s = *sp;
    s.dbg("conv bwd begin", cw.name);
    if (act != ACT_NONE) launch_act_bwd(s, y, act, slope, act == ACT_PRELU ? s.gr(cw.slope) : nullptr);
#ifdef DF_DEV
    static const bool overlap = df::dev_getenv("DF_TRAIN_OVERLAP") != nullptr;
    s.keep_wgrad_ws = overlap && need_dx;
    bool acc_early = false;
    if (s.keep_wgrad_ws) acc_early = s.grad_of(x);
    const size_t mark_layer = s.off;
#endif
    {
      std::vector<WgradSeg> segs;
      if (flat) segs.push_back(WgradSeg{(int)x->rows(), 1, 1, 1, 1, 0, 0});
      else for (int i = 0; i < nb; ++i) segs.push_back(WgradSeg{li->B[i], li->H[i], li->W[i], lo->H[i], lo->W[i], li->off[i], lo->off[i]});
      ConvParams f = (*plan)[0];
      f.in = x->v.d;
      wgrad(s, f, segs, y->g, s.gr(cw.name, cw.woff), cw.bias.empty() ? nullptr : s.gr(cw.bias, cw.boff));
    }
    if (need_dx) {
#ifdef DF_DEV
      const bool acc = s.keep_wgrad_ws ? acc_early : s.grad_of(x);
#else
      const bool acc = s.grad_of(x);
#endif
      if (flat) dgrad(s, (*plan)[0], y->g, x->g, s.pf(cw.name, cw.woff), acc);
      else {
        std::vector<int> direct;
        for (int i = 0; i < nb; ++i) {
          bool on_f4 = false;
          for (int j : *f4) on_f4 |= j == i;
          if (!on_f4) direct.push_back(i);
        }
        if (stride != 1) {
          const int kk = k * k * cin;
          const size_t mark = s.off;
          float *dcol = s.f((size_t)lo->rows * kk);
          ConvParams q;
          q.in = y->g.d; q.B = (int)lo->rows; q.Cin = cout; q.in_ld = y->g.ld;
          q.wgt = s.pf(cw.name, cw.woff);
          q.out = dcol; q.Cout = kk; q.out_ld = kk;
          q.splitk_ws = s.splitk; q.splitk_ws_bytes = s.splitk_bytes;
          s.gemm(GK_DGRAD, q);
          if (s.live())
            for (const BTab &t : make_tabs(li, lo))
              hipLaunchKernelGGL(col2im_multi_kernel, dim3(nblk(tab_rows(t) * (cin / 4))), dim3(TB), 0, s.st, dcol, x->g.d, x->g.ld, cin, k, stride, pad, dil,
                                 acc ? 1 : 0, t);
          s.off = mark;
        } else if (direct.size() == 1)
          for (int i : direct) dgrad(s, (*plan)[i], rows_view(y->g, lo->off[i]), rows_view(x->g, li->off[i]), s.pf(cw.name, cw.woff), acc);
        else if (!direct.empty()) {
          const ConvParams &f = (*plan)[0];
          ConvParams q;
          q.in = y->g.d; q.Cin = f.Cout; q.in_ld = y->g.ld;
          q.wgt = s.pf(cw.name, cw.woff);
          q.out = x->g.d; q.Cout = f.Cin; q.out_ld = x->g.ld;
          q.KH = f.KH; q.KW = f.KW; q.stride = 1; q.dil = f.dil; q.pad = f.dil * (f.KH - 1) - f.pad;
          if (acc) { q.res = x->g.d; q.res_ld = x->g.ld; }
          std::vector<WgradSeg> segs;
          for (int i : direct) segs.push_back(WgradSeg{lo->B[i], lo->H[i], lo->W[i], li->H[i], li->W[i], lo->off[i], li->off[i]});
          s.gemm_multi(GK_DGRAD, q, segs);
        }
        wino_pass(s, y->g, cout, s.dry || !wino_ok ? nullptr : s.t->wino_buf + wit->second.bwd, x->g, cin, acc ? x->g.d : nullptr, x->g.ld, ACT_NONE, GK_DGRAD);
      }
    }
#ifdef DF_DEV
    if (s.keep_wgrad_ws) {
      if (s.live() && s.side) hipStreamWaitEvent(s.st, s.ev_join, 0);
      s.off = mark_layer;
      s.keep_wgrad_ws = false;
    }
#endif
    if (res) {
      if (!res->gset) { res->g = y->g; res->gset = true; }
      else if (s.live()) hipLaunchKernelGGL(add2d_kernel, dim3(nblk(y->rows() * (y->C / 4))), dim3(TB), 0, s.st, res->g.d, res->g.ld, y->g.d, y->g.ld,
                                            y->rows(), y->C / 4);
    }
  });
  return y;
}

Act *slice(Step &s, Act *a, int c0, int C) {
  s.acts.emplace_back();
  Act *v = &s.acts.back();
  *v = *a;
  v->v.d = a->v.d + c0;
  v->C = C;
  v->g = View{};
  v->gset = false;
  return v;
}

int check_flips(Trainer &t, const float *P, long version, hipStream_t st) {
  if (!t.wflip || (t.wino_floats && !t.wino_buf))
    return set_error(DF_ERR_STATE, "trainer: created without a device (no arena for the data gradients' weight copies)");
  if (t.flip_version == version && t.flip_src == P && version >= 0) return DF_OK;
  if (t.flip_tiles)
    hipLaunchKernelGGL(flip_tiles_kernel, dim3(t.flip_ntiles), dim3(256), 0, st, P, t.wflip, t.flip_tiles, (int)t.flips.size());
  else if (t.flip_tab)
    hipLaunchKernelGGL(flip_all_kernel, dim3(nblk(t.flip_total, 8192)), dim3(TB), 0, st, P, t.wflip, t.flip_tab, (int)t.flips.size(), t.flip_total);
  else
    for (const Trainer::Flip &f : t.flips)
      hipLaunchKernelGGL(flip_kernel, dim3(nblk((long)f.O * f.T * f.I * f.Z, 1024)), dim3(TB), 0, st, P + f.off, t.wflip + f.off, f.O, f.T, f.I, f.KH, f.KW, f.Z);
  {
    WinoWTab tab;
    tab.n = 0; tab.e0[0] = 0;
    auto flush = [&]() { launch_wino4_weight_multi(P, t.wflip, t.wino_buf, tab, st); tab.n = 0; tab.e0[0] = 0; };
    auto push = [&](int O, int C, int from_b, long src, long dst) {
      if (tab.n == WINO_WMAX) flush();
      const int g = tab.n++;
      tab.O[g] = O; tab.C[g] = C; tab.from_b[g] = from_b; tab.src_off[g] = src; tab.dst_off[g] = dst;
      tab.e0[g + 1] = tab.e0[g] + (long)O * C;
    };
    for (const auto &kv : t.wino) {
      const Trainer::Wino &w = kv.second;
      push(w.O, w.I, 0, (long)w.w_off, (long)w.fwd);
      push(w.I, w.O, 1, (long)w.w_off, (long)w.bwd);
    }
    flush();
  }
  t.flip_version = version;
  t.flip_src = P;
  return check_launch("trainer: weight flips");
}

struct PoseNetIO {
  int nb;
  const int *B, *H, *W;
  const float *const *img;
  int M;
  const float *cloud, *target, *model_points;
  const int64_t *choose, *obj;
  const int *symmetric;
  float w;
  int dropout;
  unsigned seed;
  float *loss, *dis, *new_points, *new_target;
  float *out_r, *out_t, *out_c, *emb;
};

Act *basic_block(Step &s, Act *x, int cin, const std::string &base, int planes, int stride, int dil, bool has_ds, Act *out_into = nullptr) {
  Act *t = conv(s, x, cin, ConvW{base + "conv1.weight"}, planes, 3, stride, dil, dil, ACT_RELU);
  Act *res = x;
  if (has_ds) res = conv(s, x, cin, ConvW{base + "downsample.0.weight"}, planes, 1, stride, 0, 1, ACT_NONE);
  return conv(s, t, planes, ConvW{base + "conv2.weight"}, planes, 3, 1, dil, dil, ACT_RELU, res, out_into);
}

Act *dropout2d(Step &s, Act *a, float p, unsigned seed) {
  const Lv *lv = a->lv;
  float *scale = s.f((size_t)lv->frames * a->C);
  Act *o = s.act(lv, a->C);
  const std::vector<BTab> tabs = make_tabs(lv);
  if (s.live()) {
    s.fail(df_dropout2d_mask(scale, (int64_t)lv->frames * a->C, seed, p, s.st));
    for (const BTab &t : tabs)
      hipLaunchKernelGGL(channel_scale_multi_kernel, dim3(nblk(tab_rows(t) * (a->C / 4))), dim3(TB), 0, s.st, a->v.d, a->v.ld, scale, o->v.d, o->v.ld, a->C / 4, t);
  }
  Step *sp = &s;
  s.tape.push_back([=]() {
    Step &s = *sp;
    s.grad_of(a);
    if (s.live())
      for (const BTab &t : tabs)
        hipLaunchKernelGGL(channel_scale_multi_kernel, dim3(nblk(tab_rows(t) * (a->C / 4))), dim3(TB), 0, s.st, o->g.d, o->g.ld, scale, a->g.d, a->g.ld, a->C / 4, t);
  });
  return o;
}

Act *upconv(Step &s, Act *x, const std::string &base, int cin, int cout) {
  const Lv *li = x->lv;
  const int nb = li->nb();
  Act *y = s.act(li, 9 * cout);
  const ConvW cw{base + "conv.1.weight"};
  ConvParams p = flat_params(x, cin, s.p(cw.name), nullptr, y, ACT_NONE);
  p.splitk_ws = s.splitk; p.splitk_ws_bytes = s.splitk_bytes;
  s.gemm(GK_FWD, p);
  Lv up;
  for (int i = 0; i < nb; ++i) up.push(li->B[i], 2 * li->H[i], 2 * li->W[i]);
  const Lv *lo = s.level(up);
  Act *o = s.act(lo, cout);
  if (s.live())
    for (int i = 0; i < nb; ++i)
      s.fail(launch_upconv_gather(y->v.d + li->off[i] * 9 * cout, s.p(base + "conv.1.bias"), s.p(base + "conv.2.weight"), o->v.d + lo->off[i] * cout, li->B[i],
                                  li->H[i], li->W[i], cout, s.st));
  Step *sp = &s;
  s.tape.push_back([=]() {
    Step &s = *sp;
    launch_act_bwd(s, o, ACT_PRELU, s.p(base + "conv.2.weight"), s.gr(base + "conv.2.weight"));
    {
      const long rows = o->rows();
      const int nbk = (int)((rows + 255) / 256);
      float *part = s.f((size_t)nbk * cout);
      if (s.live()) {
        hipLaunchKernelGGL(colsum_obj_kernel, dim3((cout + 31) / 32, nbk), dim3(256), 0, s.st, o->g.d, o->g.ld, part, 256, cout, rows);
        hipLaunchKernelGGL(colsum_obj_kernel, dim3((cout + 31) / 32, 1), dim3(256), 0, s.st, part, cout, s.gr(base + "conv.1.bias"), nbk, cout, (long)nbk, 1);
      }
    }
    s.grad_of(y);
    if (s.live())
      for (const BTab &t : make_tabs(li))
        hipLaunchKernelGGL(upconv_gather_bwd_multi_kernel, dim3(nblk(tab_rows(t) * 9 * (cout / 4))), dim3(TB), 0, s.st, o->g.d, y->g.d, cout, t);
    wgrad(s, p, y->g, s.gr(cw.name), nullptr);
    const bool acc = s.grad_of(x);
    dgrad(s, p, y->g, x->g, s.pf(cw.name), acc);
  });
  return o;
}

void posenet_step(Step &s, const PoseNetIO &io) {
  Trainer &t = *s.t;
  const std::string C = CNN;
  int B = 0;
  for (int i = 0; i < io.nb; ++i) B += io.B[i];
  const int nb = io.nb, N = t.N, Npad = round_up(N, 128), rows = B * Npad;
  s.splitk_bytes = (size_t)32 << 20;
  s.splitk = static_cast<float *>(s.bytes(s.splitk_bytes));
  if (!t.splitk) { s.splitk = nullptr; s.splitk_bytes = 0; }
  Step *sp = &s;

  Lv limg;
  for (int i = 0; i < nb; ++i) limg.push(io.B[i], io.H[i], io.W[i]);
  Act *img4 = s.act(s.level(limg), 4);
  if (s.live())
    for (int i = 0; i < nb; ++i) launch_nchw3_to_nhwc4(io.img[i], img4->v.d + img4->lv->off[i] * 4, io.B[i], io.H[i], io.W[i], s.st);
  Act *stem = conv(s, img4, 4, ConvW{C + "feats.conv1.weight"}, 64, 7, 2, 3, 1, ACT_RELU, nullptr, nullptr, false);
  Lv lpool;
  for (int i = 0; i < nb; ++i) lpool.push(io.B[i], conv_out(stem->lv->H[i], 3, 2, 1, 1), conv_out(stem->lv->W[i], 3, 2, 1, 1));
  Act *x = s.act(s.level(lpool), 64);
  {
    const Lv *ls = stem->lv, *lx = x->lv;
    if (s.live())
      for (int i = 0; i < nb; ++i)
        launch_maxpool3s2(stem->v.d + ls->off[i] * 64, x->v.d + lx->off[i] * 64, ls->B[i], ls->H[i], ls->W[i], 64, lx->H[i], lx->W[i], s.st);
    Act *xp = x;
    s.tape.push_back([=]() {
      Step &s = *sp;
      s.grad_of(stem);
      if (s.live())
        for (const BTab &t : make_tabs(ls, lx))
          hipLaunchKernelGGL(maxpool3s2_bwd_multi_kernel, dim3(nblk(tab_rows(t) * 16)), dim3(TB), 0, s.st, stem->v.d, xp->g.d, stem->g.d, 64, t);
    });
  }
  int cin = 64;
  const int planes_of[4] = {64, 128, 256, 512}, stride_of[4] = {1, 2, 1, 1}, dil_of[4] = {1, 1, 2, 4};
  Act *cat = nullptr;
  for (int li = 1; li <= 4; ++li) {
    const int planes = planes_of[li - 1];
    const std::string base = C + "feats.layer" + std::to_string(li) + ".";
    x = basic_block(s, x, cin, base + "0.", planes, stride_of[li - 1], 1, cin != planes || stride_of[li - 1] != 1);
    Act *into = nullptr;
    if (li == 4) {
      cat = s.act(x->lv, 2560);
      into = slice(s, cat, 2048, 512);
    }
    x = basic_block(s, x, planes, base + "1.", planes, 1, dil_of[li - 1], false, into);
    cin = planes;
  }
  const Lv *l8 = cat->lv;
  Act *feat = x;
  float *pyr = s.f((size_t)4 * B * 36 * 512);
  if (s.live())
    for (int i = 0; i < nb; ++i)
      launch_psp_pool(feat->v.d + l8->off[i] * feat->v.ld, feat->v.ld, 0, pyr, l8->B[i], l8->H[i], l8->W[i], 512, s.st, B, l8->b0[i]);
  struct Stages { Act *pooled[4], *z[4]; };
  auto stg = std::make_shared<Stages>();
  const std::vector<BTab> tabs8 = make_tabs(l8);
  s.tape.push_back([=]() {
    Step &s = *sp;
    const bool acc = s.grad_of(feat);
    Ptr4 dy;
    for (int si = 0; si < 4; ++si) dy.p[si] = stg->pooled[si]->g.d;
    if (s.live())
      for (const BTab &t : tabs8)
        hipLaunchKernelGGL(pool_bwd_all_kernel, dim3(nblk(tab_rows(t) * 128)), dim3(TB), 0, s.st, dy, feat->g.d, feat->g.ld, 128, acc ? 1 : 0, t);
  });
  for (int si = 0; si < 4; ++si) {
    const int sz = si == 0 ? 1 : si == 1 ? 2 : si == 2 ? 3 : 6;
    stg->pooled[si] = s.act((long)B * sz * sz, 512, pyr + (size_t)si * B * 36 * 512, 512);
    stg->z[si] = conv(s, stg->pooled[si], 512, ConvW{C + "psp.stages." + std::to_string(si) + ".1.weight"}, 512, 1, 1, 0, 1, ACT_NONE);
  }
  {
    Ptr4 z;
    for (int si = 0; si < 4; ++si) z.p[si] = stg->z[si]->v.d;
    if (s.live())
      for (const BTab &t : tabs8)
        hipLaunchKernelGGL(bilinear_fwd_all_kernel, dim3(nblk(tab_rows(t) * 4 * 128)), dim3(TB), 0, s.st, z, cat->v.d, cat->v.ld, 128, t);
  }
  s.tape.push_back([=]() {
    Step &s = *sp;
    MPtr4 dz;
    for (int si = 0; si < 4; ++si) { s.grad_of(stg->z[si]); dz.p[si] = stg->z[si]->g.d; }
    if (s.live())
      for (const BTab &t : tabs8)
        hipLaunchKernelGGL(bilinear_bwd_all_kernel, dim3((unsigned)std::min<long>((long)tab_frames(t) * 50 * 16, 65535L * 16)), dim3(TB), 0, s.st, cat->g.d, cat->g.ld,
                           dz, tab_frames(t), 128, t);
  });
  s.tape.push_back([=]() {
// ... 557 lines not shown
```

densefusion_amd/csrc/wino.h:

```cpp
#pragma once
#include "igemm.h"

namespace df {

constexpr int WINO_MAXB = 16;
struct WinoTab { int n; int H[WINO_MAXB], W[WINO_MAXB], TH[WINO_MAXB], TW[WINO_MAXB], blocks[WINO_MAXB + 1]; long T[WINO_MAXB], row0[WINO_MAXB], t0[WINO_MAXB]; };
struct WinoGeom { int TH, TW; long T; };
WinoGeom wino_geom(int B, int H, int W, int dil, int m = 2);
int wino_route(int H, int W, int dil, int Cin, int Cout);
void launch_wino_weight(const float *w_packed , float *U , int O, int C, hipStream_t st, int m = 2);
constexpr int WINO_WMAX = 32;
struct WinoWTab { int n; int O[WINO_WMAX], C[WINO_WMAX], from_b[WINO_WMAX]; long src_off[WINO_WMAX], dst_off[WINO_WMAX], e0[WINO_WMAX + 1]; };
void launch_wino4_weight_multi(const float *src_a, const float *src_b, float *dst, const WinoWTab &tab, hipStream_t st);
void launch_wino_input(const float *x, int in_ld, int in_coff, float *V , int B, int H, int W, int C, int dil,
                       hipStream_t st, long Ttot = 0, long t0 = 0, int m = 2);
void launch_wino_output(const float *M , float *out, int out_ld, int out_coff, const float *bias, const float *res,
                        int res_ld, int res_coff, int act, int B, int H, int W, int C, int dil, hipStream_t st, long Ttot = 0, long t0 = 0,
                        int m = 2);

void launch_wino4_input_multi(const float *x, int in_ld, float *V, int nb, const int *B, const int *H, const int *W, const long *row0, const long *t0,
                              int C, int dil, long Ttot, hipStream_t st);
void launch_wino4_output_multi(const float *M, float *out, int out_ld, const float *res, int res_ld, int act, int nb, const int *B, const int *H,
                               const int *W, const long *row0, const long *t0, int C, int dil, long Ttot, hipStream_t st);

}
```

densefusion_amd/csrc/wino.hip:

```cpp
#include "wino.h"

namespace df {
namespace {

constexpr int WB = 256;

struct TileId { int b, ry, rx, ty, tx; };

__device__ __forceinline__ TileId tile_of(int t, int d, int TH, int TW) {
  TileId r;
  r.tx = t % TW; t /= TW;
  r.ty = t % TH; t /= TH;
  r.rx = t % d; t /= d;
  r.ry = t % d;
  r.b = t / d;
  return r;
}

__device__ __forceinline__ float4 f4add(float4 a, float4 b) { return make_float4(a.x + b.x, a.y + b.y, a.z + b.z, a.w + b.w); }
__device__ __forceinline__ float4 f4sub(float4 a, float4 b) { return make_float4(a.x - b.x, a.y - b.y, a.z - b.z, a.w - b.w); }

__global__ __launch_bounds__(WB) void wino_weight_kernel(const float *__restrict__ w, float *__restrict__ U, int O, int C) {
  const long n = (long)O * C;
  for (long e = (long)blockIdx.x * WB + threadIdx.x; e < n; e += (long)gridDim.x * WB) {
    const int o = (int)(e / C), c = (int)(e % C);
    double g[3][3], t[4][3];
#pragma unroll
    for (int i = 0; i < 3; ++i)
#pragma unroll
      for (int j = 0; j < 3; ++j) g[i][j] = (double)w[((size_t)o * 9 + i * 3 + j) * C + c];
#pragma unroll
    for (int j = 0; j < 3; ++j) {
      t[0][j] = g[0][j];
      t[1][j] = 0.5 * (g[0][j] + g[1][j] + g[2][j]);
      t[2][j] = 0.5 * (g[0][j] - g[1][j] + g[2][j]);
      t[3][j] = g[2][j];
    }
#pragma unroll
    for (int i = 0; i < 4; ++i) {
      const double u0 = t[i][0], u1 = 0.5 * (t[i][0] + t[i][1] + t[i][2]), u2 = 0.5 * (t[i][0] - t[i][1] + t[i][2]), u3 = t[i][2];
      U[((size_t)(i * 4 + 0) * O + o) * C + c] = (float)u0;
      U[((size_t)(i * 4 + 1) * O + o) * C + c] = (float)u1;
      U[((size_t)(i * 4 + 2) * O + o) * C + c] = (float)u2;
      U[((size_t)(i * 4 + 3) * O + o) * C + c] = (float)u3;
    }
  }
}

__global__ __launch_bounds__(WB) void wino_input_kernel(const float *__restrict__ x, int in_ld, int in_coff, float *__restrict__ V, int H,
                                                        int W, int C, int d, int TH, int TW, long T, long Ttot, long t0) {
  const int c4n = C >> 2;
  const long total = T * c4n;
  for (long e = (long)blockIdx.x * WB + threadIdx.x; e < total; e += (long)gridDim.x * WB) {
    const int c = (int)(e % c4n) << 2;
    const long t = e / c4n;
    const TileId id = tile_of((int)t, d, TH, TW);
    const int y0 = id.ry + d * (2 * id.ty - 1), x0 = id.rx + d * (2 * id.tx - 1);
    float4 p[4][4];
#pragma unroll
    for (int i = 0; i < 4; ++i) {
      const int y = y0 + d * i;
#pragma unroll
      for (int j = 0; j < 4; ++j) {
        const int xx = x0 + d * j;
        const bool ok = (unsigned)y < (unsigned)H && (unsigned)xx < (unsigned)W;
        p[i][j] = ok ? *reinterpret_cast<const float4 *>(x + ((size_t)(id.b * H + y) * W + xx) * in_ld + in_coff + c)
                     : make_float4(0.f, 0.f, 0.f, 0.f);
      }
    }
    float4 r[4][4];
#pragma unroll
    for (int j = 0; j < 4; ++j) {
      r[0][j] = f4sub(p[0][j], p[2][j]);
      r[1][j] = f4add(p[1][j], p[2][j]);
      r[2][j] = f4sub(p[2][j], p[1][j]);
      r[3][j] = f4sub(p[1][j], p[3][j]);
    }
#pragma unroll
    for (int i = 0; i < 4; ++i) {
      float4 *dst = reinterpret_cast<float4 *>(V + ((size_t)(i * 4) * Ttot + t0 + t) * C + c);
      const size_t zs = (size_t)Ttot * C / 4;
      dst[0] = f4sub(r[i][0], r[i][2]);
      dst[zs] = f4add(r[i][1], r[i][2]);
      dst[2 * zs] = f4sub(r[i][2], r[i][1]);
      dst[3 * zs] = f4sub(r[i][1], r[i][3]);
    }
  }
}

__global__ __launch_bounds__(WB) void wino_output_kernel(const float *__restrict__ Mz, float *__restrict__ out, int out_ld, int out_coff,
                                                         const float *__restrict__ bias, const float *__restrict__ res, int res_ld,
                                                         int res_coff, int act, int H, int W,
                                                         int C, int d, int TH, int TW, long T, long Ttot, long t0) {
  const int c4n = C >> 2;
  const long total = T * c4n;
  for (long e = (long)blockIdx.x * WB + threadIdx.x; e < total; e += (long)gridDim.x * WB) {
    const int c = (int)(e % c4n) << 2;
    const long t = e / c4n;
    const TileId id = tile_of((int)t, d, TH, TW);
    const int oy = id.ry + d * 2 * id.ty, ox = id.rx + d * 2 * id.tx;
    if (oy >= H || ox >= W) continue;
    const size_t zs = (size_t)Ttot * C / 4;
    const float4 *src = reinterpret_cast<const float4 *>(Mz + (size_t)(t0 + t) * C + c);
    float4 s0[4], s1[4];
#pragma unroll
    for (int j = 0; j < 4; ++j) {
      const float4 m0 = src[(0 * 4 + j) * zs], m1 = src[(1 * 4 + j) * zs], m2 = src[(2 * 4 + j) * zs], m3 = src[(3 * 4 + j) * zs];
      s0[j] = f4add(f4add(m0, m1), m2);
      s1[j] = f4sub(f4sub(m1, m2), m3);
    }
    float4 y[2][2];
    y[0][0] = f4add(f4add(s0[0], s0[1]), s0[2]);
    y[0][1] = f4sub(f4sub(s0[1], s0[2]), s0[3]);
    y[1][0] = f4add(f4add(s1[0], s1[1]), s1[2]);
    y[1][1] = f4sub(f4sub(s1[1], s1[2]), s1[3]);
#pragma unroll
    for (int a = 0; a < 2; ++a) {
      const int yy = oy + d * a;
      if (yy >= H) continue;
#pragma unroll
      for (int b2 = 0; b2 < 2; ++b2) {
        const int xx = ox + d * b2;
        if (xx >= W) continue;
        const size_t pix = (size_t)(id.b * H + yy) * W + xx;
        float4 v = y[a][b2];
        if (bias) v = f4add(v, *reinterpret_cast<const float4 *>(bias + c));
        if (res) v = f4add(v, *reinterpret_cast<const float4 *>(res + pix * res_ld + res_coff + c));
        if (act == ACT_RELU) v = make_float4(fmaxf(v.x, 0.f), fmaxf(v.y, 0.f), fmaxf(v.z, 0.f), fmaxf(v.w, 0.f));
        *reinterpret_cast<float4 *>(out + pix * out_ld + out_coff + c) = v;
      }
    }
  }
}

__device__ __forceinline__ float4 f4s(float a, float4 v) { return make_float4(a * v.x, a * v.y, a * v.z, a * v.w); }

__device__ __forceinline__ void bt6(const float4 d0, const float4 d1, const float4 d2, const float4 d3, const float4 d4, const float4 d5,
                                    float4 *r, int stride) {
  const float4 a = f4add(d4, f4s(-2.f, d2)), b = f4s(1.5f, f4sub(d3, d1));
  r[0 * stride] = f4add(f4add(d0, a), b);
  r[1 * stride] = f4add(f4sub(d4, d1), f4add(f4s(0.5f, d2), f4s(2.5f, d3)));
  r[2 * stride] = f4add(f4add(d4, d1), f4add(f4s(-2.5f, d2), f4s(0.5f, d3)));
  r[3 * stride] = f4add(f4sub(d4, d2), f4s(2.f, f4sub(d3, d1)));
  r[4 * stride] = f4add(f4sub(d4, d2), f4s(0.5f, f4sub(d1, d3)));
  r[5 * stride] = f4add(f4add(d5, f4add(d1, f4s(-2.f, d3))), f4s(1.5f, f4sub(d4, d2)));
  (void)a; (void)b;
}

__global__ __launch_bounds__(WB) void wino4_weight_kernel(const float *__restrict__ w, float *__restrict__ U, int O, int C) {
  const long n = (long)O * C;
  const double G[6][3] = {{1, 0, 0}, {1. / 3, 1. / 3, 1. / 3}, {-1. / 3, 1. / 3, -1. / 3}, {-16. / 15, -8. / 15, -4. / 15},
                          {1. / 15, -2. / 15, 4. / 15}, {0, 0, 1}};
  for (long e = (long)blockIdx.x * WB + threadIdx.x; e < n; e += (long)gridDim.x * WB) {
    const int o = (int)(e / C), c = (int)(e % C);
    double g[3][3], t[6][3];
#pragma unroll
    for (int i = 0; i < 3; ++i)
#pragma unroll
      for (int j = 0; j < 3; ++j) g[i][j] = (double)w[((size_t)o * 9 + i * 3 + j) * C + c];
#pragma unroll
    for (int i = 0; i < 6; ++i)
#pragma unroll
      for (int j = 0; j < 3; ++j) t[i][j] = G[i][0] * g[0][j] + G[i][1] * g[1][j] + G[i][2] * g[2][j];
#pragma unroll
    for (int i = 0; i < 6; ++i)
#pragma unroll
      for (int j = 0; j < 6; ++j)
        U[((size_t)(i * 6 + j) * O + o) * C + c] = (float)(t[i][0] * G[j][0] + t[i][1] * G[j][1] + t[i][2] * G[j][2]);
  }
}

__global__ __launch_bounds__(WB) void wino4_weight_multi_kernel(const float *__restrict__ src_a, const float *__restrict__ src_b, float *__restrict__ dst,
                                                                const WinoWTab tab) {
  const double G[6][3] = {{1, 0, 0}, {1. / 3, 1. / 3, 1. / 3}, {-1. / 3, 1. / 3, -1. / 3}, {-16. / 15, -8. / 15, -4. / 15},
                          {1. / 15, -2. / 15, 4. / 15}, {0, 0, 1}};
  const long n = tab.e0[tab.n];
  for (long e0 = (long)blockIdx.x * WB + threadIdx.x; e0 < n; e0 += (long)gridDim.x * WB) {
    int sgi = 0;
    while (sgi + 1 < tab.n && e0 >= tab.e0[sgi + 1]) ++sgi;
    const long e = e0 - tab.e0[sgi];
    const int O = tab.O[sgi], C = tab.C[sgi];
    const float *w = (tab.from_b[sgi] ? src_b : src_a) + tab.src_off[sgi];
    float *U = dst + tab.dst_off[sgi];
    const int o = (int)(e / C), c = (int)(e % C);
    double g[3][3], t[6][3];
#pragma unroll
    for (int i = 0; i < 3; ++i)
#pragma unroll
      for (int j = 0; j < 3; ++j) g[i][j] = (double)w[((size_t)o * 9 + i * 3 + j) * C + c];
#pragma unroll
    for (int i = 0; i < 6; ++i)
#pragma unroll
      for (int j = 0; j < 3; ++j) t[i][j] = G[i][0] * g[0][j] + G[i][1] * g[1][j] + G[i][2] * g[2][j];
#pragma unroll
    for (int i = 0; i < 6; ++i)
#pragma unroll
      for (int j = 0; j < 6; ++j)
        U[((size_t)(i * 6 + j) * O + o) * C + c] = (float)(t[i][0] * G[j][0] + t[i][1] * G[j][1] + t[i][2] * G[j][2]);
  }
}

__device__ __forceinline__ void wino4_input_body(const float *__restrict__ x, int in_ld, int in_coff, float *__restrict__ V, int H, int W, int C, int d,
                                                 int TH, int TW, long T, long Ttot, long t0, long e_begin, long e_step) {
  const int c4n = C >> 2;
  const long total = T * c4n;
  for (long e = e_begin; e < total; e += e_step) {
    const int c = (int)(e % c4n) << 2;
    const long t = e / c4n;
    const TileId id = tile_of((int)t, d, TH, TW);
    const int y0 = id.ry + d * (4 * id.ty - 1), x0 = id.rx + d * (4 * id.tx - 1);
    float4 r[6][6];
#pragma unroll
    for (int j = 0; j < 6; ++j) {
      const int xx = x0 + d * j;
      float4 p[6];
#pragma unroll
      for (int i = 0; i < 6; ++i) {
        const int y = y0 + d * i;
        const bool ok = (unsigned)y < (unsigned)H && (unsigned)xx < (unsigned)W;
        p[i] = ok ? *reinterpret_cast<const float4 *>(x + ((size_t)(id.b * H + y) * W + xx) * in_ld + in_coff + c)
                  : make_float4(0.f, 0.f, 0.f, 0.f);
      }
      bt6(p[0], p[1], p[2], p[3], p[4], p[5], &r[0][j], 6);
    }
    const size_t zs = (size_t)Ttot * C / 4;
    float4 *dst = reinterpret_cast<float4 *>(V + ((size_t)t0 + t) * C + c);
#pragma unroll
    for (int i = 0; i < 6; ++i) {
      float4 v[6];
      bt6(r[i][0], r[i][1], r[i][2], r[i][3], r[i][4], r[i][5], v, 1);
#pragma unroll
      for (int j = 0; j < 6; ++j) dst[(size_t)(i * 6 + j) * zs] = v[j];
    }
  }
}

__device__ __forceinline__ void at6(const float4 m0, const float4 m1, const float4 m2, const float4 m3, const float4 m4, const float4 m5,
                                    float4 *y, int stride) {
  const float4 s12 = f4add(m1, m2), d12 = f4sub(m1, m2);
  y[0 * stride] = f4add(f4add(m0, s12), f4add(m3, m4));
  y[1 * stride] = f4add(d12, f4add(f4s(0.5f, m3), f4s(-2.f, m4)));
  y[2 * stride] = f4add(s12, f4add(f4s(0.25f, m3), f4s(4.f, m4)));
  y[3 * stride] = f4add(f4add(d12, m5), f4add(f4s(0.125f, m3), f4s(-8.f, m4)));
}

__global__ __launch_bounds__(WB) void wino4_input_kernel(const float *__restrict__ x, int in_ld, int in_coff, float *__restrict__ V, int H,
                                                         int W, int C, int d, int TH, int TW, long T, long Ttot, long t0) {
  wino4_input_body(x, in_ld, in_coff, V, H, W, C, d, TH, TW, T, Ttot, t0, (long)blockIdx.x * WB + threadIdx.x, (long)gridDim.x * WB);
}
__global__ __launch_bounds__(WB) void wino4_input_multi_kernel(const float *__restrict__ x, int in_ld, float *__restrict__ V, int C, int d, long Ttot,
                                                               const WinoTab tab) {
  int k = 0;
  while (k + 1 < tab.n && (int)blockIdx.x >= tab.blocks[k + 1]) ++k;
  wino4_input_body(x + tab.row0[k] * in_ld, in_ld, 0, V, tab.H[k], tab.W[k], C, d, tab.TH[k], tab.TW[k], tab.T[k], Ttot, tab.t0[k],
                   (long)((int)blockIdx.x - tab.blocks[k]) * WB + threadIdx.x, (long)(tab.blocks[k + 1] - tab.blocks[k]) * WB);
}

__device__ __forceinline__ void wino4_output_body(const float *__restrict__ Mz, float *__restrict__ out, int out_ld, int out_coff,
                                                  const float *__restrict__ bias, const float *__restrict__ res, int res_ld, int res_coff, int act, int H,
                                                  int W, int C, int d, int TH, int TW, long T, long Ttot, long t0, long e_begin, long e_step) {
  const int c4n = C >> 2;
  const long total = T * c4n;
  for (long e = e_begin; e < total; e += e_step) {
    const int c = (int)(e % c4n) << 2;
    const long t = e / c4n;
    const TileId id = tile_of((int)t, d, TH, TW);
    const int oy = id.ry + d * 4 * id.ty, ox = id.rx + d * 4 * id.tx;
    if (oy >= H || ox >= W) continue;
    const size_t zs = (size_t)Ttot * C / 4;
    const float4 *src = reinterpret_cast<const float4 *>(Mz + ((size_t)t0 + t) * C + c);
    float4 s[4][6];
#pragma unroll
    for (int j = 0; j < 6; ++j)
      at6(src[(size_t)(0 * 6 + j) * zs], src[(size_t)(1 * 6 + j) * zs], src[(size_t)(2 * 6 + j) * zs], src[(size_t)(3 * 6 + j) * zs],
          src[(size_t)(4 * 6 + j) * zs], src[(size_t)(5 * 6 + j) * zs], &s[0][j], 6);
    float4 bv = make_float4(0.f, 0.f, 0.f, 0.f);
    if (bias) bv = *reinterpret_cast<const float4 *>(bias + c);
#pragma unroll
    for (int a = 0; a < 4; ++a) {
      const int yy = oy + d * a;
      if (yy >= H) continue;
      float4 y[4];
      at6(s[a][0], s[a][1], s[a][2], s[a][3], s[a][4], s[a][5], y, 1);
#pragma unroll
      for (int b2 = 0; b2 < 4; ++b2) {
        const int xx = ox + d * b2;
        if (xx >= W) continue;
        const size_t pix = (size_t)(id.b * H + yy) * W + xx;
        float4 v = y[b2];
        if (bias) v = f4add(v, bv);
        if (res) v = f4add(v, *reinterpret_cast<const float4 *>(res + pix * res_ld + res_coff + c));
        if (act == ACT_RELU) v = make_float4(fmaxf(v.x, 0.f), fmaxf(v.y, 0.f), fmaxf(v.z, 0.f), fmaxf(v.w, 0.f));
        *reinterpret_cast<float4 *>(out + pix * out_ld + out_coff + c) = v;
      }
    }
  }
}

__global__ __launch_bounds__(WB) void wino4_output_kernel(const float *__restrict__ Mz, float *__restrict__ out, int out_ld, int out_coff,
                                                          const float *__restrict__ bias, const float *__restrict__ res, int res_ld,
                                                          int res_coff, int act, int H, int W, int C, int d, int TH, int TW, long T,
                                                          long Ttot, long t0) {
  wino4_output_body(Mz, out, out_ld, out_coff, bias, res, res_ld, res_coff, act, H, W, C, d, TH, TW, T, Ttot, t0,
                    (long)blockIdx.x * WB + threadIdx.x, (long)gridDim.x * WB);
}
__global__ __launch_bounds__(WB) void wino4_output_multi_kernel(const float *__restrict__ Mz, float *__restrict__ out, int out_ld, const float *__restrict__ res,
                                                                int res_ld, int act, int C, int d, long Ttot, const WinoTab tab) {
  int k = 0;
  while (k + 1 < tab.n && (int)blockIdx.x >= tab.blocks[k + 1]) ++k;
  wino4_output_body(Mz, out + tab.row0[k] * out_ld, out_ld, 0, nullptr, res ? res + tab.row0[k] * res_ld : nullptr, res_ld, 0, act, tab.H[k], tab.W[k], C,
                    d, tab.TH[k], tab.TW[k], tab.T[k], Ttot, tab.t0[k], (long)((int)blockIdx.x - tab.blocks[k]) * WB + threadIdx.x,
                    (long)(tab.blocks[k + 1] - tab.blocks[k]) * WB);
}

inline unsigned blocks_for(long n) {
  const long b = (n + WB - 1) / WB;
  return (unsigned)(b < 1 ? 1 : (b > 65535L * 16 ? 65535L * 16 : b));
}

}

WinoGeom wino_geom(int B, int H, int W, int dil, int m) {
  WinoGeom g;
  g.TH = ((H + dil - 1) / dil + m - 1) / m;
  g.TW = ((W + dil - 1) / dil + m - 1) / m;
  g.T = (long)B * dil * dil * g.TH * g.TW;
  return g;
}

int wino_route(int H, int W, int dil, int Cin, int Cout) {
  if (Cin < 128 || Cin % 4 || Cout % 4) return 0;
  const double px = (double)H * W, cc = (double)Cin * Cout;
  const double rate = Cin >= 512 ? 144e12 : Cin >= 256 ? 128e12 : 100e12;
  double best = 18.0 * cc / 145e12;
  int route = 0;
  for (int m = 2; m <= 4; m += 2) {
    const double n2 = (double)(m + 2) * (m + 2);
    const double per_px = n2 * (double)wino_geom(1, H, W, dil, m).T / px;
    const double t = 2.0 * per_px * cc / rate + 4.0 * ((1.0 + per_px) * Cin + (per_px + 2.0) * Cout) / 4.0e12;
    if (t < 0.9 * best) { best = t / 0.9; route = m; }
  }
  return route;
}

void launch_wino_weight(const float *w_packed, float *U, int O, int C, hipStream_t st, int m) {
  if (m == 4) hipLaunchKernelGGL(wino4_weight_kernel, dim3(blocks_for((long)O * C)), dim3(WB), 0, st, w_packed, U, O, C);
  else hipLaunchKernelGGL(wino_weight_kernel, dim3(blocks_for((long)O * C)), dim3(WB), 0, st, w_packed, U, O, C);
}

void launch_wino4_weight_multi(const float *src_a, const float *src_b, float *dst, const WinoWTab &tab, hipStream_t st) {
  if (tab.n <= 0) return;
  hipLaunchKernelGGL(wino4_weight_multi_kernel, dim3(blocks_for(tab.e0[tab.n])), dim3(WB), 0, st, src_a, src_b, dst, tab);
}

void launch_wino_input(const float *x, int in_ld, int in_coff, float *V, int B, int H, int W, int C, int dil, hipStream_t st, long Ttot,
                       long t0, int m) {
  const WinoGeom g = wino_geom(B, H, W, dil, m);
  if (Ttot <= 0) { Ttot = g.T; t0 = 0; }
  if (m == 4)
    hipLaunchKernelGGL(wino4_input_kernel, dim3(blocks_for(g.T * (C / 4))), dim3(WB), 0, st, x, in_ld, in_coff, V, H, W, C, dil, g.TH, g.TW, g.T,
                       Ttot, t0);
  else
    hipLaunchKernelGGL(wino_input_kernel, dim3(blocks_for(g.T * (C / 4))), dim3(WB), 0, st, x, in_ld, in_coff, V, H, W, C, dil, g.TH, g.TW, g.T,
                       Ttot, t0);
}

void launch_wino_output(const float *M, float *out, int out_ld, int out_coff, const float *bias, const float *res, int res_ld, int res_coff,
                        int act, int B, int H, int W, int C, int dil, hipStream_t st, long Ttot, long t0, int m) {
  const WinoGeom g = wino_geom(B, H, W, dil, m);
  if (Ttot <= 0) { Ttot = g.T; t0 = 0; }
  if (m == 4)
    hipLaunchKernelGGL(wino4_output_kernel, dim3(blocks_for(g.T * (C / 4))), dim3(WB), 0, st, M, out, out_ld, out_coff, bias, res, res_ld,
                       res_coff, act, H, W, C, dil, g.TH, g.TW, g.T, Ttot, t0);
  else
    hipLaunchKernelGGL(wino_output_kernel, dim3(blocks_for(g.T * (C / 4))), dim3(WB), 0, st, M, out, out_ld, out_coff, bias, res, res_ld,
                       res_coff, act, H, W, C, dil, g.TH, g.TW, g.T, Ttot, t0);
}

static WinoTab make_tab(int n, const int *B, const int *H, const int *W, const long *row0, const long *t0, int C, int dil) {
  WinoTab tab;
  tab.n = n;
  tab.blocks[0] = 0;
  for (int k = 0; k < n; ++k) {
    const WinoGeom g = wino_geom(B[k], H[k], W[k], dil, 4);
    tab.H[k] = H[k]; tab.W[k] = W[k]; tab.TH[k] = g.TH; tab.TW[k] = g.TW; tab.T[k] = g.T; tab.row0[k] = row0[k]; tab.t0[k] = t0[k];
    tab.blocks[k + 1] = tab.blocks[k] + (int)blocks_for(g.T * (C / 4));
  }
  return tab;
}

void launch_wino4_input_multi(const float *x, int in_ld, float *V, int nb, const int *B, const int *H, const int *W, const long *row0, const long *t0,
                              int C, int dil, long Ttot, hipStream_t st) {
  for (int k0 = 0; k0 < nb; k0 += WINO_MAXB) {
    const int n = nb - k0 < WINO_MAXB ? nb - k0 : WINO_MAXB;
    const WinoTab tab = make_tab(n, B + k0, H + k0, W + k0, row0 + k0, t0 + k0, C, dil);
    hipLaunchKernelGGL(wino4_input_multi_kernel, dim3(tab.blocks[n]), dim3(WB), 0, st, x, in_ld, V, C, dil, Ttot, tab);
  }
}

void launch_wino4_output_multi(const float *M, float *out, int out_ld, const float *res, int res_ld, int act, int nb, const int *B, const int *H,
                               const int *W, const long *row0, const long *t0, int C, int dil, long Ttot, hipStream_t st) {
  for (int k0 = 0; k0 < nb; k0 += WINO_MAXB) {
    const int n = nb - k0 < WINO_MAXB ? nb - k0 : WINO_MAXB;
    const WinoTab tab = make_tab(n, B + k0, H + k0, W + k0, row0 + k0, t0 + k0, C, dil);
    hipLaunchKernelGGL(wino4_output_multi_kernel, dim3(tab.blocks[n]), dim3(WB), 0, st, M, out, out_ld, res, res_ld, act, C, dil, Ttot, tab);
  }
}

}
```

Baseline: 8693.

## Add F(3x3,3x3) Winograd route and tighten dilated tile geometry per phase

Adds a Winograd F(3,3) variant (5x5 transform tiles) with weight, input and output kernels. It also changes tile geometry so each dilation phase gets its own tile count, which drops the wasted out-of-bounds tiles and the per-tile bounds check. The default router now weighs m=2, 3 and 4 using the exact tile counts, so more feature-map sizes can pick the transform with the least padding waste. The cost is extra weight-transform memory (25*O*I per layer), more kernel variants, and more integer index arithmetic per tile.

```diff
diff --git a/densefusion_amd/csrc/engine.hip b/densefusion_amd/csrc/engine.hip
--- a/densefusion_amd/csrc/engine.hip
+++ b/densefusion_amd/csrc/engine.hip
@@ -197,9 +197,11 @@
       hipLaunchKernelGGL(pack_oihw_kernel, dim3(256), dim3(256), 0, 0, n.stage, dst, O, I, HW, Ipad);
     }
     if (e == hipSuccess && key.find("feats.layer") != std::string::npos && HW == 9 && I >= 128 && I % 4 == 0 && O % 4 == 0) {
-      float *U = dev_alloc(n, key + ".wino", (size_t)16 * O * I), *U4 = dev_alloc(n, key + ".wino4", (size_t)36 * O * I);
-      if (!U || !U4) return set_error(DF_ERR_LAUNCH, "load_param: hipMalloc failed");
+      float *U = dev_alloc(n, key + ".wino", (size_t)16 * O * I), *U3 = dev_alloc(n, key + ".wino3", (size_t)25 * O * I);
+      float *U4 = dev_alloc(n, key + ".wino4", (size_t)36 * O * I);
+      if (!U || !U3 || !U4) return set_error(DF_ERR_LAUNCH, "load_param: hipMalloc failed");
       launch_wino_weight(dst, U, O, I, 0, 2);
+      launch_wino_weight(dst, U3, O, I, 0, 3);
       launch_wino_weight(dst, U4, O, I, 0, 4);
     }
     if (e == hipSuccess && (key.find(".up_1.") != std::string::npos || key.find(".up_2.") != std::string::npos) && HW == 9) {
@@ -365,8 +367,9 @@
 static int wino_route_for(int H, int W, int dil, int ci, int co) {
   static const bool off = df::dev_getenv("DF_NO_WINOGRAD") != nullptr;
   static const int force = df::dev_getenv("DF_WINOGRAD_TILE") ? atoi(df::dev_getenv("DF_WINOGRAD_TILE")) : 0;
+  static const bool v4 = df::dev_getenv("DF_WINO_ROUTE_V4") != nullptr;
   if (off) return 0;
-  const int r = wino_route(H, W, dil, ci, co);
+  const int r = v4 ? wino_route_v4(H, W, dil, ci, co) : wino_route(H, W, dil, ci, co);
   return (r && force == 2) ? 2 : r;
 }
 
@@ -436,18 +439,19 @@
 
   auto conv3x3 = [&](const float *in, const Level &li, int ci, const std::string &key, float *out, const Level &lo, int co, int stride, int dil,
                      const float *res) {
-    std::vector<int> ws[2];
+    std::vector<int> ws[3];
     for (int i = 0; i < nb; ++i) {
       const int route = stride == 1 ? wino_route_for(li.h[i], li.w[i], dil, ci, co) : 0;
-      if (route) { ws[route == 4].push_back(i); continue; }
+      if (route) { ws[route - 2].push_back(i); continue; }
       ConvParams p = conv2d(in + li.off[i] * ci, gs[i].B, li.h[i], li.w[i], ci, ci, c.w(key), nullptr, out + lo.off[i] * co, lo.h[i], lo.w[i], co,
                             co, 0, 3, stride, dil, dil, ACT_RELU);
       if (res) { p.res = res + lo.off[i] * co; p.res_ld = co; }
       c.conv(p);
     }
-    for (int r = 0; r < 2; ++r) {
+    static const char *const wkey[3] = {".wino", ".wino3", ".wino4"};
+    for (int r = 0; r < 3; ++r) {
       if (ws[r].empty()) continue;
-      const int m = r ? 4 : 2, nz = (m + 2) * (m + 2);
+      const int m = r + 2, nz = (m + 2) * (m + 2);
       std::vector<long> t0;
       long T = 0;
       for (int i : ws[r]) { t0.push_back(T); T += wino_geom(gs[i].B, li.h[i], li.w[i], dil, m).T; }
@@ -458,21 +462,22 @@
       for (int i : ws[r]) { tB.push_back(gs[i].B); tH.push_back(li.h[i]); tW.push_back(li.w[i]); trow.push_back(li.off[i]); }
       const int nw = (int)ws[r].size();
       static const bool per_bucket = df::dev_getenv("DF_WINO_PER_BUCKET") != nullptr;
-      if (m == 4 && !per_bucket) {
-        if (c.live()) launch_wino4_input_multi(in, ci, V, nw, tB.data(), tH.data(), tW.data(), trow.data(), t0.data(), ci, dil, T, c.st);
+      if (m > 2 && !per_bucket) {
+        if (c.live()) launch_wino_input_multi(in, ci, V, nw, tB.data(), tH.data(), tW.data(), trow.data(), t0.data(), ci, dil, T, c.st, m);
       } else {
         for (size_t j = 0; j < ws[r].size(); ++j) {
           const int i = ws[r][j];
           if (c.live()) launch_wino_input(in + li.off[i] * ci, ci, 0, V, gs[i].B, li.h[i], li.w[i], ci, dil, c.st, T, t0[j], m);
         }
       }
-      ConvParams p = point_gemm(V, ci, 0, ci, c.w(key + (r ? ".wino4" : ".wino")), nullptr, M, co, 0, co, (int)T, ACT_NONE);
+      ConvParams p = point_gemm(V, ci, 0, ci, c.w(key + wkey[r]), nullptr, M, co, 0, co, (int)T, ACT_NONE);
       p.zcount = nz; p.z_in_coff = T * ci; p.z_wgt = (long)co * ci; p.z_out_coff = T * co;
       double px = 0;
       for (int i : ws[r]) px += (double)gs[i].B * li.h[i] * li.w[i];
       c.conv(p, px / ((double)(m * m) * (double)T));
-      if (m == 4 && !per_bucket) {
-        if (c.live()) launch_wino4_output_multi(M, out, co, res, co, ACT_RELU, nw, tB.data(), tH.data(), tW.data(), trow.data(), t0.data(), co, dil, T, c.st);
+      if (m > 2 && !per_bucket) {
+        if (c.live())
+          launch_wino_output_multi(M, out, co, res, co, ACT_RELU, nw, tB.data(), tH.data(), tW.data(), trow.data(), t0.data(), co, dil, T, c.st, m);
       } else {
         for (size_t j = 0; j < ws[r].size(); ++j) {
           const int i = ws[r][j];
@@ -1111,7 +1116,7 @@
 
 extern "C" size_t df_conv3x3_winograd_tile_scratch_bytes(const df_conv_desc *d, int tile) {
   if (wino_desc_ok(d, "conv3x3_winograd_scratch_bytes") != DF_OK) return 0;
-  if (tile != 2 && tile != 4) { set_error(DF_ERR_ARG, "conv3x3_winograd: tile must be 2 or 4"); return 0; }
+  if (tile < 2 || tile > 4) { set_error(DF_ERR_ARG, "conv3x3_winograd: tile must be 2, 3 or 4"); return 0; }
   const WinoGeom g = wino_geom(d->B, d->H, d->W, d->dil, tile);
   const size_t nz = (size_t)(tile + 2) * (tile + 2);
   return (nz * d->Cout * d->Cin + nz * g.T * d->Cin + nz * g.T * d->Cout) * sizeof(float);
@@ -1120,7 +1125,7 @@
 extern "C" int df_conv3x3_winograd_tile_nhwc(const df_conv_desc *d, int tile, void *scratch, size_t scratch_bytes, df_stream_t stream) {
   int rc = wino_desc_ok(d, "conv3x3_winograd_nhwc");
   if (rc != DF_OK) return rc;
-  if (tile != 2 && tile != 4) return set_error(DF_ERR_ARG, "conv3x3_winograd: tile must be 2 or 4");
+  if (tile < 2 || tile > 4) return set_error(DF_ERR_ARG, "conv3x3_winograd: tile must be 2, 3 or 4");
   if (!d->in || !d->wgt || !d->out || !scratch) return set_error(DF_ERR_ARG, "conv3x3_winograd_nhwc: null pointer");
   if (scratch_bytes < df_conv3x3_winograd_tile_scratch_bytes(d, tile)) return set_error(DF_ERR_WORKSPACE, "conv3x3_winograd_nhwc: scratch too small");
   const WinoGeom g = wino_geom(d->B, d->H, d->W, d->dil, tile);
diff --git a/densefusion_amd/csrc/train.hip b/densefusion_amd/csrc/train.hip
--- a/densefusion_amd/csrc/train.hip
+++ b/densefusion_amd/csrc/train.hip
@@ -1477,7 +1477,7 @@
       p.prelu = slope;
       p.splitk_ws = s.splitk; p.splitk_ws_bytes = s.splitk_bytes;
       plan->push_back(p);
-      if (wino_ok && wino_route(li->H[i], li->W[i], dil, cin, cout) == 4) { f4->push_back(i); continue; }
+      if (wino_ok && wino_route_v4(li->H[i], li->W[i], dil, cin, cout) == 4) { f4->push_back(i); continue; }
       if (first_direct < 0) first_direct = i;
       direct.push_back(WgradSeg{li->B[i], li->H[i], li->W[i], lo->H[i], lo->W[i], li->off[i], lo->off[i]});
     }
@@ -1503,13 +1503,13 @@
     float *V = s.f((size_t)36 * T * ci), *M = s.f((size_t)36 * T * co);
     if (s.live()) {
       const int nw = (int)f4->size();
-      launch_wino4_input_multi(in.d, in.ld, V, nw, tB.data(), tH.data(), tW.data(), trow.data(), t0.data(), ci, dil, T, s.st);
+      launch_wino_input_multi(in.d, in.ld, V, nw, tB.data(), tH.data(), tW.data(), trow.data(), t0.data(), ci, dil, T, s.st, 4);
       ConvParams q;
       q.in = V; q.wgt = U; q.out = M;
       q.B = (int)T; q.Cin = ci; q.in_ld = ci; q.Cout = co; q.out_ld = co;
       q.zcount = 36; q.z_in_coff = T * ci; q.z_wgt = (long)co * ci; q.z_out_coff = T * co;
       s.gemm(kind, q);
-      launch_wino4_output_multi(M, out.d, out.ld, rs, rs_ld, a, nw, tB.data(), tH.data(), tW.data(), trow.data(), t0.data(), co, dil, T, s.st);
+      launch_wino_output_multi(M, out.d, out.ld, rs, rs_ld, a, nw, tB.data(), tH.data(), tW.data(), trow.data(), t0.data(), co, dil, T, s.st, 4);
     }
     s.off = mark;
   };
diff --git a/densefusion_amd/csrc/wino.h b/densefusion_amd/csrc/wino.h
--- a/densefusion_amd/csrc/wino.h
+++ b/densefusion_amd/csrc/wino.h
@@ -4,10 +4,12 @@
 namespace df {
 
 constexpr int WINO_MAXB = 16;
-struct WinoTab { int n; int H[WINO_MAXB], W[WINO_MAXB], TH[WINO_MAXB], TW[WINO_MAXB], blocks[WINO_MAXB + 1]; long T[WINO_MAXB], row0[WINO_MAXB], t0[WINO_MAXB]; };
-struct WinoGeom { int TH, TW; long T; };
+struct WinoDim { int nhi, thi, tlo, n; };
+struct WinoGeom { WinoDim h, w; long T; };
+struct WinoTab { int n; int H[WINO_MAXB], W[WINO_MAXB], blocks[WINO_MAXB + 1]; WinoGeom g[WINO_MAXB]; long row0[WINO_MAXB], t0[WINO_MAXB]; };
 WinoGeom wino_geom(int B, int H, int W, int dil, int m = 2);
 int wino_route(int H, int W, int dil, int Cin, int Cout);
+int wino_route_v4(int H, int W, int dil, int Cin, int Cout);
 void launch_wino_weight(const float *w_packed , float *U , int O, int C, hipStream_t st, int m = 2);
 constexpr int WINO_WMAX = 32;
 struct WinoWTab { int n; int O[WINO_WMAX], C[WINO_WMAX], from_b[WINO_WMAX]; long src_off[WINO_WMAX], dst_off[WINO_WMAX], e0[WINO_WMAX + 1]; };
@@ -18,9 +20,9 @@
                         int res_ld, int res_coff, int act, int B, int H, int W, int C, int dil, hipStream_t st, long Ttot = 0, long t0 = 0,
                         int m = 2);
 
-void launch_wino4_input_multi(const float *x, int in_ld, float *V, int nb, const int *B, const int *H, const int *W, const long *row0, const long *t0,
-                              int C, int dil, long Ttot, hipStream_t st);
-void launch_wino4_output_multi(const float *M, float *out, int out_ld, const float *res, int res_ld, int act, int nb, const int *B, const int *H,
-                               const int *W, const long *row0, const long *t0, int C, int dil, long Ttot, hipStream_t st);
+void launch_wino_input_multi(const float *x, int in_ld, float *V, int nb, const int *B, const int *H, const int *W, const long *row0, const long *t0,
+                             int C, int dil, long Ttot, hipStream_t st, int m);
+void launch_wino_output_multi(const float *M, float *out, int out_ld, const float *res, int res_ld, int act, int nb, const int *B, const int *H,
+                              const int *W, const long *row0, const long *t0, int C, int dil, long Ttot, hipStream_t st, int m);
 
 }
diff --git a/densefusion_amd/csrc/wino.hip b/densefusion_amd/csrc/wino.hip
--- a/densefusion_amd/csrc/wino.hip
+++ b/densefusion_amd/csrc/wino.hip
@@ -7,13 +7,24 @@
 
 struct TileId { int b, ry, rx, ty, tx; };
 
-__device__ __forceinline__ TileId tile_of(int t, int d, int TH, int TW) {
+__device__ __forceinline__ void dim_of(int r, const WinoDim D, int &phase, int &tile) {
+  const int s = D.nhi * D.thi;
+  if (r < s) {
+    phase = r / D.thi; tile = r - phase * D.thi;
+  } else {
+    const int q = r - s, k = q / D.tlo;
+    phase = D.nhi + k; tile = q - k * D.tlo;
+  }
+}
+
+__device__ __forceinline__ TileId tile_of(long t, const WinoGeom &g) {
   TileId r;
-  r.tx = t % TW; t /= TW;
-  r.ty = t % TH; t /= TH;
-  r.rx = t % d; t /= d;
-  r.ry = t % d;
-  r.b = t / d;
+  const int tc = (int)(t % g.w.n);
+  t /= g.w.n;
+  const int tr = (int)(t % g.h.n);
+  r.b = (int)(t / g.h.n);
+  dim_of(tr, g.h, r.ry, r.ty);
+  dim_of(tc, g.w, r.rx, r.tx);
   return r;
 }
 
@@ -48,13 +59,13 @@
 }
 
 __global__ __launch_bounds__(WB) void wino_input_kernel(const float *__restrict__ x, int in_ld, int in_coff, float *__restrict__ V, int H,
-                                                        int W, int C, int d, int TH, int TW, long T, long Ttot, long t0) {
+                                                        int W, int C, int d, const WinoGeom g, long Ttot, long t0) {
   const int c4n = C >> 2;
-  const long total = T * c4n;
+  const long total = g.T * c4n;
   for (long e = (long)blockIdx.x * WB + threadIdx.x; e < total; e += (long)gridDim.x * WB) {
     const int c = (int)(e % c4n) << 2;
     const long t = e / c4n;
-    const TileId id = tile_of((int)t, d, TH, TW);
+    const TileId id = tile_of(t, g);
     const int y0 = id.ry + d * (2 * id.ty - 1), x0 = id.rx + d * (2 * id.tx - 1);
     float4 p[4][4];
 #pragma unroll
@@ -91,15 +102,14 @@
 __global__ __launch_bounds__(WB) void wino_output_kernel(const float *__restrict__ Mz, float *__restrict__ out, int out_ld, int out_coff,
                                                          const float *__restrict__ bias, const float *__restrict__ res, int res_ld,
                                                          int res_coff, int act, int H, int W,
-                                                         int C, int d, int TH, int TW, long T, long Ttot, long t0) {
+                                                         int C, int d, const WinoGeom g, long Ttot, long t0) {
   const int c4n = C >> 2;
-  const long total = T * c4n;
+  const long total = g.T * c4n;
   for (long e = (long)blockIdx.x * WB + threadIdx.x; e < total; e += (long)gridDim.x * WB) {
     const int c = (int)(e % c4n) << 2;
     const long t = e / c4n;
-    const TileId id = tile_of((int)t, d, TH, TW);
+    const TileId id = tile_of(t, g);
     const int oy = id.ry + d * 2 * id.ty, ox = id.rx + d * 2 * id.tx;
-    if (oy >= H || ox >= W) continue;
     const size_t zs = (size_t)Ttot * C / 4;
     const float4 *src = reinterpret_cast<const float4 *>(Mz + (size_t)(t0 + t) * C + c);
     float4 s0[4], s1[4];
@@ -201,13 +211,13 @@
 }
 
 __device__ __forceinline__ void wino4_input_body(const float *__restrict__ x, int in_ld, int in_coff, float *__restrict__ V, int H, int W, int C, int d,
-                                                 int TH, int TW, long T, long Ttot, long t0, long e_begin, long e_step) {
+                                                 const WinoGeom g, long Ttot, long t0, long e_begin, long e_step) {
   const int c4n = C >> 2;
-  const long total = T * c4n;
+  const long total = g.T * c4n;
   for (long e = e_begin; e < total; e += e_step) {
     const int c = (int)(e % c4n) << 2;
     const long t = e / c4n;
-    const TileId id = tile_of((int)t, d, TH, TW);
+    const TileId id = tile_of(t, g);
     const int y0 = id.ry + d * (4 * id.ty - 1), x0 = id.rx + d * (4 * id.tx - 1);
     float4 r[6][6];
 #pragma unroll
@@ -245,28 +255,27 @@
 }
 
 __global__ __launch_bounds__(WB) void wino4_input_kernel(const float *__restrict__ x, int in_ld, int in_coff, float *__restrict__ V, int H,
-                                                         int W, int C, int d, int TH, int TW, long T, long Ttot, long t0) {
-  wino4_input_body(x, in_ld, in_coff, V, H, W, C, d, TH, TW, T, Ttot, t0, (long)blockIdx.x * WB + threadIdx.x, (long)gridDim.x * WB);
+                                                         int W, int C, int d, const WinoGeom g, long Ttot, long t0) {
+  wino4_input_body(x, in_ld, in_coff, V, H, W, C, d, g, Ttot, t0, (long)blockIdx.x * WB + threadIdx.x, (long)gridDim.x * WB);
 }
 __global__ __launch_bounds__(WB) void wino4_input_multi_kernel(const float *__restrict__ x, int in_ld, float *__restrict__ V, int C, int d, long Ttot,
                                                                const WinoTab tab) {
   int k = 0;
   while (k + 1 < tab.n && (int)blockIdx.x >= tab.blocks[k + 1]) ++k;
-  wino4_input_body(x + tab.row0[k] * in_ld, in_ld, 0, V, tab.H[k], tab.W[k], C, d, tab.TH[k], tab.TW[k], tab.T[k], Ttot, tab.t0[k],
+  wino4_input_body(x + tab.row0[k] * in_ld, in_ld, 0, V, tab.H[k], tab.W[k], C, d, tab.g[k], Ttot, tab.t0[k],
                    (long)((int)blockIdx.x - tab.blocks[k]) * WB + threadIdx.x, (long)(tab.blocks[k + 1] - tab.blocks[k]) * WB);
 }
 
 __device__ __forceinline__ void wino4_output_body(const float *__restrict__ Mz, float *__restrict__ out, int out_ld, int out_coff,
                                                   const float *__restrict__ bias, const float *__restrict__ res, int res_ld, int res_coff, int act, int H,
-                                                  int W, int C, int d, int TH, int TW, long T, long Ttot, long t0, long e_begin, long e_step) {
+                                                  int W, int C, int d, const WinoGeom g, long Ttot, long t0, long e_begin, long e_step) {
   const int c4n = C >> 2;
-  const long total = T * c4n;
+  const long total = g.T * c4n;
   for (long e = e_begin; e < total; e += e_step) {
     const int c = (int)(e % c4n) << 2;
     const long t = e / c4n;
-    const TileId id = tile_of((int)t, d, TH, TW);
+    const TileId id = tile_of(t, g);
     const int oy = id.ry + d * 4 * id.ty, ox = id.rx + d * 4 * id.tx;
-    if (oy >= H || ox >= W) continue;
     const size_t zs = (size_t)Ttot * C / 4;
     const float4 *src = reinterpret_cast<const float4 *>(Mz + ((size_t)t0 + t) * C + c);
     float4 s[4][6];
@@ -299,9 +308,8 @@
 
 __global__ __launch_bounds__(WB) void wino4_output_kernel(const float *__restrict__ Mz, float *__restrict__ out, int out_ld, int out_coff,
                                                           const float *__restrict__ bias, const float *__restrict__ res, int res_ld,
-                                                          int res_coff, int act, int H, int W, int C, int d, int TH, int TW, long T,
-                                                          long Ttot, long t0) {
-  wino4_output_body(Mz, out, out_ld, out_coff, bias, res, res_ld, res_coff, act, H, W, C, d, TH, TW, T, Ttot, t0,
+                                                          int res_coff, int act, int H, int W, int C, int d, const WinoGeom g, long Ttot, long t0) {
+  wino4_output_body(Mz, out, out_ld, out_coff, bias, res, res_ld, res_coff, act, H, W, C, d, g, Ttot, t0,
                     (long)blockIdx.x * WB + threadIdx.x, (long)gridDim.x * WB);
 }
 __global__ __launch_bounds__(WB) void wino4_output_multi_kernel(const float *__restrict__ Mz, float *__restrict__ out, int out_ld, const float *__restrict__ res,
@@ -309,7 +317,146 @@
   int k = 0;
   while (k + 1 < tab.n && (int)blockIdx.x >= tab.blocks[k + 1]) ++k;
   wino4_output_body(Mz, out + tab.row0[k] * out_ld, out_ld, 0, nullptr, res ? res + tab.row0[k] * res_ld : nullptr, res_ld, 0, act, tab.H[k], tab.W[k], C,
-                    d, tab.TH[k], tab.TW[k], tab.T[k], Ttot, tab.t0[k], (long)((int)blockIdx.x - tab.blocks[k]) * WB + threadIdx.x,
+                    d, tab.g[k], Ttot, tab.t0[k], (long)((int)blockIdx.x - tab.blocks[k]) * WB + threadIdx.x,
+                    (long)(tab.blocks[k + 1] - tab.blocks[k]) * WB);
+}
+
+__device__ __forceinline__ void bt5(const float4 d0, const float4 d1, const float4 d2, const float4 d3, const float4 d4, float4 *r, int stride) {
+  const float4 d31 = f4sub(d3, d1);
+  r[0 * stride] = f4add(f4sub(d0, d2), f4s(2.f, d31));
+  r[1 * stride] = f4add(f4sub(d2, d1), f4s(2.f, d3));
+  r[2 * stride] = f4add(f4add(d1, f4s(2.f, d3)), f4s(-3.f, d2));
+  r[3 * stride] = d31;
+  r[4 * stride] = f4add(f4sub(d1, d3), f4s(2.f, f4sub(d4, d2)));
+}
+
+__device__ __forceinline__ void at5(const float4 m0, const float4 m1, const float4 m2, const float4 m3, const float4 m4, float4 *y, int stride) {
+  const float4 s12 = f4add(m1, m2), d12 = f4sub(m1, m2);
+  y[0 * stride] = f4add(f4add(m0, s12), m3);
+  y[1 * stride] = f4add(d12, f4s(0.5f, m3));
+  y[2 * stride] = f4add(f4add(s12, f4s(0.25f, m3)), m4);
+}
+
+__global__ __launch_bounds__(WB) void wino3_weight_kernel(const float *__restrict__ w, float *__restrict__ U, int O, int C) {
+  const long n = (long)O * C;
+  const double G[5][3] = {{1, 0, 0}, {.5, .5, .5}, {-1. / 6, 1. / 6, -1. / 6}, {-8. / 3, -4. / 3, -2. / 3}, {0, 0, .5}};
+  for (long e = (long)blockIdx.x * WB + threadIdx.x; e < n; e += (long)gridDim.x * WB) {
+    const int o = (int)(e / C), c = (int)(e % C);
+    double g[3][3], t[5][3];
+#pragma unroll
+    for (int i = 0; i < 3; ++i)
+#pragma unroll
+      for (int j = 0; j < 3; ++j) g[i][j] = (double)w[((size_t)o * 9 + i * 3 + j) * C + c];
+#pragma unroll
+    for (int i = 0; i < 5; ++i)
+#pragma unroll
+      for (int j = 0; j < 3; ++j) t[i][j] = G[i][0] * g[0][j] + G[i][1] * g[1][j] + G[i][2] * g[2][j];
+#pragma unroll
+    for (int i = 0; i < 5; ++i)
+#pragma unroll
+      for (int j = 0; j < 5; ++j)
+        U[((size_t)(i * 5 + j) * O + o) * C + c] = (float)(t[i][0] * G[j][0] + t[i][1] * G[j][1] + t[i][2] * G[j][2]);
+  }
+}
+
+__device__ __forceinline__ void wino3_input_body(const float *__restrict__ x, int in_ld, int in_coff, float *__restrict__ V, int H, int W, int C, int d,
+                                                 const WinoGeom g, long Ttot, long t0, long e_begin, long e_step) {
+  const int c4n = C >> 2;
+  const long total = g.T * c4n;
+  for (long e = e_begin; e < total; e += e_step) {
+    const int c = (int)(e % c4n) << 2;
+    const long t = e / c4n;
+    const TileId id = tile_of(t, g);
+    const int y0 = id.ry + d * (3 * id.ty - 1), x0 = id.rx + d * (3 * id.tx - 1);
+    float4 r[5][5];
+#pragma unroll
+    for (int j = 0; j < 5; ++j) {
+      const int xx = x0 + d * j;
+      float4 p[5];
+#pragma unroll
+      for (int i = 0; i < 5; ++i) {
+        const int y = y0 + d * i;
+        const bool ok = (unsigned)y < (unsigned)H && (unsigned)xx < (unsigned)W;
+        p[i] = ok ? *reinterpret_cast<const float4 *>(x + ((size_t)(id.b * H + y) * W + xx) * in_ld + in_coff + c)
+                  : make_float4(0.f, 0.f, 0.f, 0.f);
+      }
+      bt5(p[0], p[1], p[2], p[3], p[4], &r[0][j], 5);
+    }
+    const size_t zs = (size_t)Ttot * C / 4;
+    float4 *dst = reinterpret_cast<float4 *>(V + ((size_t)t0 + t) * C + c);
+#pragma unroll
+    for (int i = 0; i < 5; ++i) {
+      float4 v[5];
+      bt5(r[i][0], r[i][1], r[i][2], r[i][3], r[i][4], v, 1);
+#pragma unroll
+      for (int j = 0; j < 5; ++j) dst[(size_t)(i * 5 + j) * zs] = v[j];
+    }
+  }
+}
+
+__device__ __forceinline__ void wino3_output_body(const float *__restrict__ Mz, float *__restrict__ out, int out_ld, int out_coff,
+                                                  const float *__restrict__ bias, const float *__restrict__ res, int res_ld, int res_coff, int act, int H,
+                                                  int W, int C, int d, const WinoGeom g, long Ttot, long t0, long e_begin, long e_step) {
+  const int c4n = C >> 2;
+  const long total = g.T * c4n;
+  for (long e = e_begin; e < total; e += e_step) {
+    const int c = (int)(e % c4n) << 2;
+    const long t = e / c4n;
+    const TileId id = tile_of(t, g);
+    const int oy = id.ry + d * 3 * id.ty, ox = id.rx + d * 3 * id.tx;
+    const size_t zs = (size_t)Ttot * C / 4;
+    const float4 *src = reinterpret_cast<const float4 *>(Mz + ((size_t)t0 + t) * C + c);
+    float4 s[3][5];
+#pragma unroll
+    for (int j = 0; j < 5; ++j)
+      at5(src[(size_t)(0 * 5 + j) * zs], src[(size_t)(1 * 5 + j) * zs], src[(size_t)(2 * 5 + j) * zs], src[(size_t)(3 * 5 + j) * zs],
+          src[(size_t)(4 * 5 + j) * zs], &s[0][j], 5);
+    float4 bv = make_float4(0.f, 0.f, 0.f, 0.f);
+    if (bias) bv = *reinterpret_cast<const float4 *>(bias + c);
+#pragma unroll
+    for (int a = 0; a < 3; ++a) {
+      const int yy = oy + d * a;
+      if (yy >= H) continue;
+      float4 y[3];
+      at5(s[a][0], s[a][1], s[a][2], s[a][3], s[a][4], y, 1);
+#pragma unroll
+      for (int b2 = 0; b2 < 3; ++b2) {
+        const int xx = ox + d * b2;
+        if (xx >= W) continue;
+        const size_t pix = (size_t)(id.b * H + yy) * W + xx;
+        float4 v = y[b2];
+        if (bias) v = f4add(v, bv);
+        if (res) v = f4add(v, *reinterpret_cast<const float4 *>(res + pix * res_ld + res_coff + c));
+        if (act == ACT_RELU) v = make_float4(fmaxf(v.x, 0.f), fmaxf(v.y, 0.f), fmaxf(v.z, 0.f), fmaxf(v.w, 0.f));
+        *reinterpret_cast<float4 *>(out + pix * out_ld + out_coff + c) = v;
+      }
+    }
+  }
+}
+
+__global__ __launch_bounds__(WB) void wino3_input_kernel(const float *__restrict__ x, int in_ld, int in_coff, float *__restrict__ V, int H,
+                                                         int W, int C, int d, const WinoGeom g, long Ttot, long t0) {
+  wino3_input_body(x, in_ld, in_coff, V, H, W, C, d, g, Ttot, t0, (long)blockIdx.x * WB + threadIdx.x, (long)gridDim.x * WB);
+}
+__global__ __launch_bounds__(WB) void wino3_input_multi_kernel(const float *__restrict__ x, int in_ld, float *__restrict__ V, int C, int d, long Ttot,
+                                                               const WinoTab tab) {
+  int k = 0;
+  while (k + 1 < tab.n && (int)blockIdx.x >= tab.blocks[k + 1]) ++k;
+  wino3_input_body(x + tab.row0[k] * in_ld, in_ld, 0, V, tab.H[k], tab.W[k], C, d, tab.g[k], Ttot, tab.t0[k],
+                   (long)((int)blockIdx.x - tab.blocks[k]) * WB + threadIdx.x, (long)(tab.blocks[k + 1] - tab.blocks[k]) * WB);
+}
+__global__ __launch_bounds__(WB) void wino3_output_kernel(const float *__restrict__ Mz, float *__restrict__ out, int out_ld, int out_coff,
+                                                          const float *__restrict__ bias, const float *__restrict__ res, int res_ld,
+                                                          int res_coff, int act, int H, int W, int C, int d, const WinoGeom g, long Ttot, long t0) {
+  wino3_output_body(Mz, out, out_ld, out_coff, bias, res, res_ld, res_coff, act, H, W, C, d, g, Ttot, t0,
+                    (long)blockIdx.x * WB + threadIdx.x, (long)gridDim.x * WB);
+}
+__global__ __launch_bounds__(WB) void wino3_output_multi_kernel(const float *__restrict__ Mz, float *__restrict__ out, int out_ld, const float *__restrict__ res,
+                                                                int res_ld, int act, int C, int d, long Ttot, const WinoTab tab) {
+  int k = 0;
+  while (k + 1 < tab.n && (int)blockIdx.x >= tab.blocks[k + 1]) ++k;
+  wino3_output_body(Mz, out + tab.row0[k] * out_ld, out_ld, 0, nullptr, res ? res + tab.row0[k] * res_ld : nullptr, res_ld, 0, act, tab.H[k], tab.W[k], C,
+                    d, tab.g[k], Ttot, tab.t0[k], (long)((int)blockIdx.x - tab.blocks[k]) * WB + threadIdx.x,
                     (long)(tab.blocks[k + 1] - tab.blocks[k]) * WB);
 }
 
@@ -320,24 +467,49 @@
 
 }
 
+static WinoDim wino_dim(int H, int dil, int m) {
+  WinoDim D;
+  D.nhi = H % dil ? H % dil : dil;
+  D.thi = ((H + dil - 1) / dil + m - 1) / m;
+  D.tlo = (H / dil + m - 1) / m;
+  D.n = D.nhi * D.thi + (dil - D.nhi) * D.tlo;
+  return D;
+}
+
 WinoGeom wino_geom(int B, int H, int W, int dil, int m) {
   WinoGeom g;
-  g.TH = ((H + dil - 1) / dil + m - 1) / m;
-  g.TW = ((W + dil - 1) / dil + m - 1) / m;
-  g.T = (long)B * dil * dil * g.TH * g.TW;
+  g.h = wino_dim(H, dil, m);
+  g.w = wino_dim(W, dil, m);
+  g.T = (long)B * g.h.n * g.w.n;
   return g;
+}
+
+static double route_time(int H, int W, int Cin, int Cout, int m, double tiles) {
+  const double px = (double)H * W, cc = (double)Cin * Cout;
+  if (!m) return 18.0 * cc / 145e12;
+  const double rate = Cin >= 512 ? 144e12 : Cin >= 256 ? 128e12 : 100e12;
+  const double per_px = (double)(m + 2) * (m + 2) * tiles / px;
+  return 2.0 * per_px * cc / rate + 4.0 * ((1.0 + per_px) * Cin + (per_px + 2.0) * Cout) / 4.0e12;
 }
 
 int wino_route(int H, int W, int dil, int Cin, int Cout) {
   if (Cin < 128 || Cin % 4 || Cout % 4) return 0;
-  const double px = (double)H * W, cc = (double)Cin * Cout;
-  const double rate = Cin >= 512 ? 144e12 : Cin >= 256 ? 128e12 : 100e12;
-  double best = 18.0 * cc / 145e12;
+  double best = route_time(H, W, Cin, Cout, 0, 0);
+  int route = 0;
+  for (int m = 2; m <= 4; ++m) {
+    const double t = route_time(H, W, Cin, Cout, m, (double)wino_geom(1, H, W, dil, m).T);
+    if (t < 0.9 * best) { best = t / 0.9; route = m; }
+  }
+  return route;
+}
+
+int wino_route_v4(int H, int W, int dil, int Cin, int Cout) {
+  if (Cin < 128 || Cin % 4 || Cout % 4) return 0;
+  double best = route_time(H, W, Cin, Cout, 0, 0);
   int route = 0;
   for (int m = 2; m <= 4; m += 2) {
-    const double n2 = (double)(m + 2) * (m + 2);
-    const double per_px = n2 * (double)wino_geom(1, H, W, dil, m).T / px;
-    const double t = 2.0 * per_px * cc / rate + 4.0 * ((1.0 + per_px) * Cin + (per_px + 2.0) * Cout) / 4.0e12;
+    const double tiles = (double)dil * dil * (((H + dil - 1) / dil + m - 1) / m) * (((W + dil - 1) / dil + m - 1) / m);
+    const double t = route_time(H, W, Cin, Cout, m, tiles);
     if (t < 0.9 * best) { best = t / 0.9; route = m; }
   }
   return route;
@@ -345,6 +517,7 @@
 
 void launch_wino_weight(const float *w_packed, float *U, int O, int C, hipStream_t st, int m) {
   if (m == 4) hipLaunchKernelGGL(wino4_weight_kernel, dim3(blocks_for((long)O * C)), dim3(WB), 0, st, w_packed, U, O, C);
+  else if (m == 3) hipLaunchKernelGGL(wino3_weight_kernel, dim3(blocks_for((long)O * C)), dim3(WB), 0, st, w_packed, U, O, C);
   else hipLaunchKernelGGL(wino_weight_kernel, dim3(blocks_for((long)O * C)), dim3(WB), 0, st, w_packed, U, O, C);
 }
 
@@ -357,54 +530,54 @@
                        long t0, int m) {
   const WinoGeom g = wino_geom(B, H, W, dil, m);
   if (Ttot <= 0) { Ttot = g.T; t0 = 0; }
-  if (m == 4)
-    hipLaunchKernelGGL(wino4_input_kernel, dim3(blocks_for(g.T * (C / 4))), dim3(WB), 0, st, x, in_ld, in_coff, V, H, W, C, dil, g.TH, g.TW, g.T,
-                       Ttot, t0);
-  else
-    hipLaunchKernelGGL(wino_input_kernel, dim3(blocks_for(g.T * (C / 4))), dim3(WB), 0, st, x, in_ld, in_coff, V, H, W, C, dil, g.TH, g.TW, g.T,
-                       Ttot, t0);
+  const dim3 grid(blocks_for(g.T * (C / 4)));
+  if (m == 4) hipLaunchKernelGGL(wino4_input_kernel, grid, dim3(WB), 0, st, x, in_ld, in_coff, V, H, W, C, dil, g, Ttot, t0);
+  else if (m == 3) hipLaunchKernelGGL(wino3_input_kernel, grid, dim3(WB), 0, st, x, in_ld, in_coff, V, H, W, C, dil, g, Ttot, t0);
+  else hipLaunchKernelGGL(wino_input_kernel, grid, dim3(WB), 0, st, x, in_ld, in_coff, V, H, W, C, dil, g, Ttot, t0);
 }
 
 void launch_wino_output(const float *M, float *out, int out_ld, int out_coff, const float *bias, const float *res, int res_ld, int res_coff,
                         int act, int B, int H, int W, int C, int dil, hipStream_t st, long Ttot, long t0, int m) {
   const WinoGeom g = wino_geom(B, H, W, dil, m);
   if (Ttot <= 0) { Ttot = g.T; t0 = 0; }
+  const dim3 grid(blocks_for(g.T * (C / 4)));
   if (m == 4)
-    hipLaunchKernelGGL(wino4_output_kernel, dim3(blocks_for(g.T * (C / 4))), dim3(WB), 0, st, M, out, out_ld, out_coff, bias, res, res_ld,
-                       res_coff, act, H, W, C, dil, g.TH, g.TW, g.T, Ttot, t0);
+    hipLaunchKernelGGL(wino4_output_kernel, grid, dim3(WB), 0, st, M, out, out_ld, out_coff, bias, res, res_ld, res_coff, act, H, W, C, dil, g, Ttot, t0);
+  else if (m == 3)
+    hipLaunchKernelGGL(wino3_output_kernel, grid, dim3(WB), 0, st, M, out, out_ld, out_coff, bias, res, res_ld, res_coff, act, H, W, C, dil, g, Ttot, t0);
   else
-    hipLaunchKernelGGL(wino_output_kernel, dim3(blocks_for(g.T * (C / 4))), dim3(WB), 0, st, M, out, out_ld, out_coff, bias, res, res_ld,
-                       res_coff, act, H, W, C, dil, g.TH, g.TW, g.T, Ttot, t0);
-}
-
-static WinoTab make_tab(int n, const int *B, const int *H, const int *W, const long *row0, const long *t0, int C, int dil) {
+    hipLaunchKernelGGL(wino_output_kernel, grid, dim3(WB), 0, st, M, out, out_ld, out_coff, bias, res, res_ld, res_coff, act, H, W, C, dil, g, Ttot, t0);
+}
+
+static WinoTab make_tab(int n, const int *B, const int *H, const int *W, const long *row0, const long *t0, int C, int dil, int m) {
   WinoTab tab;
   tab.n = n;
   tab.blocks[0] = 0;
   for (int k = 0; k < n; ++k) {
-    const WinoGeom g = wino_geom(B[k], H[k], W[k], dil, 4);
-    tab.H[k] = H[k]; tab.W[k] = W[k]; tab.TH[k] = g.TH; tab.TW[k] = g.TW; tab.T[k] = g.T; tab.row0[k] = row0[k]; tab.t0[k] = t0[k];
+    const WinoGeom g = wino_geom(B[k], H[k], W[k], dil, m);
+    tab.H[k] = H[k]; tab.W[k] = W[k]; tab.g[k] = g; tab.row0[k] = row0[k]; tab.t0[k] = t0[k];
     tab.blocks[k + 1] = tab.blocks[k] + (int)blocks_for(g.T * (C / 4));
   }
   return tab;
 }
 
-void launch_wino4_input_multi(const float *x, int in_ld, float *V, int nb, const int *B, const int *H, const int *W, const long *row0, const long *t0,
-                              int C, int dil, long Ttot, hipStream_t st) {
+void launch_wino_input_multi(const float *x, int in_ld, float *V, int nb, const int *B, const int *H, const int *W, const long *row0, const long *t0,
+                             int C, int dil, long Ttot, hipStream_t st, int m) {
   for (int k0 = 0; k0 < nb; k0 += WINO_MAXB) {
     const int n = nb - k0 < WINO_MAXB ? nb - k0 : WINO_MAXB;
-    const WinoTab tab = make_tab(n, B + k0, H + k0, W + k0, row0 + k0, t0 + k0, C, dil);
-    hipLaunchKernelGGL(wino4_input_multi_kernel, dim3(tab.blocks[n]), dim3(WB), 0, st, x, in_ld, V, C, dil, Ttot, tab);
-  }
-}
-
-void launch_wino4_output_multi(const float *M, float *out, int out_ld, const float *res, int res_ld, int act, int nb, const int *B, const int *H,
-                               const int *W, const long *row0, const long *t0, int C, int dil, long Ttot, hipStream_t st) {
+    const WinoTab tab = make_tab(n, B + k0, H + k0, W + k0, row0 + k0, t0 + k0, C, dil, m);
+    hipLaunchKernelGGL(m == 3 ? wino3_input_multi_kernel : wino4_input_multi_kernel, dim3(tab.blocks[n]), dim3(WB), 0, st, x, in_ld, V, C, dil, Ttot, tab);
+  }
+}
+
+void launch_wino_output_multi(const float *M, float *out, int out_ld, const float *res, int res_ld, int act, int nb, const int *B, const int *H,
+                              const int *W, const long *row0, const long *t0, int C, int dil, long Ttot, hipStream_t st, int m) {
   for (int k0 = 0; k0 < nb; k0 += WINO_MAXB) {
     const int n = nb - k0 < WINO_MAXB ? nb - k0 : WINO_MAXB;
-    const WinoTab tab = make_tab(n, B + k0, H + k0, W + k0, row0 + k0, t0 + k0, C, dil);
-    hipLaunchKernelGGL(wino4_output_multi_kernel, dim3(tab.blocks[n]), dim3(WB), 0, st, M, out, out_ld, res, res_ld, act, C, dil, Ttot, tab);
-  }
-}
-
-}
+    const WinoTab tab = make_tab(n, B + k0, H + k0, W + k0, row0 + k0, t0 + k0, C, dil, m);
+    hipLaunchKernelGGL(m == 3 ? wino3_output_multi_kernel : wino4_output_multi_kernel, dim3(tab.blocks[n]), dim3(WB), 0, st, M, out, out_ld, res, res_ld,
+                       act, C, dil, Ttot, tab);
+  }
+}
+
+}
```

After: 8817 (median of 6 runs). 1.01x the previous value.
